# hkapp/cniic

Hardware: AMD Instinct MI355X
Metric: Mpixels/sec encode (cluster-colors K=256) (higher is better)
Workload: dtype u8/u64; 1 GPU; configs[1]: cluster-colors(256) encode of one 4096x4096 photo-like synthetic RGB image per GPU (seed 0x636E696963+2+rank), to convergence; image and stream HBM-resident; pixels_per_gpu=16777216, parallelism=1 GPU

## Files before the change

### cniic_amd/csrc/k_kmeans_persist.hip

```cpp
#include <atomic>

#include <hip/hip_ext.h>

#include "kmeans_rgbw.hpp"

namespace cniic {

constexpr int kPsThreads = 1024, kPsWaves = kPsThreads / 64;
constexpr uint32_t kPsAccWords = 5 * 256;
constexpr uint32_t kPsOffTab = kPsAccWords * 8, kPsOffS = kPsOffTab + 256 * 8;
static_assert(kPsOffCell == kPsOffS + kPsSlotsMax * kPsScap * 4, "ps_cell_bytes / kPsOffCell (kmeans_rgbw.hpp) describe this layout");

__device__ __forceinline__ uint32_t ps_xcc_id() {
    uint32_t v;
    asm volatile("s_getreg_b32 %0, hwreg(HW_REG_XCC_ID)" : "=s"(v));
    return v & 7u;
}
__device__ __forceinline__ unsigned long long ps_aread(unsigned long long *p) {
    return __hip_atomic_fetch_add(p, 0ull, __ATOMIC_RELAXED, __HIP_MEMORY_SCOPE_AGENT);
}
__device__ __forceinline__ uint32_t ps_ld(const uint32_t *p) { return __hip_atomic_load(p, __ATOMIC_RELAXED, __HIP_MEMORY_SCOPE_AGENT); }
__device__ __forceinline__ void ps_st(uint32_t *p, uint32_t v) { __hip_atomic_store(p, v, __ATOMIC_RELAXED, __HIP_MEMORY_SCOPE_AGENT); }

__device__ __forceinline__ bool ps_spin(uint32_t *word, uint32_t old, PsBar *b, unsigned long long ticks) {
    const unsigned long long t0 = wall_clock64();
    uint32_t spins = 0;
    while (ps_ld(word) == old) {
        __builtin_amdgcn_s_sleep(1);
        if ((++spins & 63u) == 0) {
            if (ps_ld(&b->abort_.v)) return false;
            if (wall_clock64() - t0 > ticks) { ps_st(&b->abort_.v, 1u); return false; }
        }
    }
    return true;
}
__device__ __forceinline__ bool ps_barrier_flat(PsBar *b, uint32_t nblocks, unsigned long long ticks) {
    const uint32_t g = ps_ld(&b->gen.v);
    if (__hip_atomic_fetch_add(&b->count.v, 1u, __ATOMIC_RELAXED, __HIP_MEMORY_SCOPE_AGENT) == nblocks - 1) {
        ps_st(&b->count.v, 0u);
        ps_st(&b->gen.v, g + 1);
        return true;
    }
    return ps_spin(&b->gen.v, g, b, ticks);
}
__device__ __forceinline__ bool ps_barrier_xcd(PsBar *b, uint32_t x, uint32_t nx_blocks, uint32_t nxcd, unsigned long long ticks) {
    const uint32_t tg = ps_ld(&b->topgen.v);
    if (__hip_atomic_fetch_add(&b->xcount[x].v, 1u, __ATOMIC_RELAXED, __HIP_MEMORY_SCOPE_AGENT) == nx_blocks - 1) {
        ps_st(&b->xcount[x].v, 0u);
        if (__hip_atomic_fetch_add(&b->top.v, 1u, __ATOMIC_RELAXED, __HIP_MEMORY_SCOPE_AGENT) == nxcd - 1) {
            ps_st(&b->top.v, 0u);
            ps_st(&b->topgen.v, tg + 1);
            return true;
        }
    }
    return ps_spin(&b->topgen.v, tg, b, ticks);
}

__global__ __launch_bounds__(1024) void k_ps_ranges(const uint32_t *__restrict__ ne_cost, const uint32_t *__restrict__ ne_count, uint32_t G, uint32_t dyn_bytes,
                                                    uint32_t *__restrict__ cb, uint32_t *__restrict__ fail) {
    const uint32_t M = *ne_count, NC = G * kPsChunks;
    const uint64_t total = ne_cost[M];
    for (uint32_t g0 = threadIdx.x; g0 <= NC; g0 += 8 * blockDim.x) {
        uint32_t a[8], b[8];
        uint64_t c_lo[8];
#pragma unroll
        for (int r = 0; r < 8; r++) {
            const uint32_t g = g0 + r * blockDim.x;
            c_lo[r] = total * min(g, NC) / NC;
            a[r] = 0; b[r] = g <= NC ? M : 0u;
        }
        bool more = true;
        while (more) {
            more = false;
            uint32_t mid[8], v[8];
#pragma unroll
            for (int r = 0; r < 8; r++) { mid[r] = (a[r] + b[r]) >> 1; v[r] = a[r] < b[r] ? ne_cost[mid[r]] : 0u; }
#pragma unroll
            for (int r = 0; r < 8; r++)
                if (a[r] < b[r]) { if (v[r] < c_lo[r]) a[r] = mid[r] + 1; else b[r] = mid[r]; more = more || a[r] < b[r]; }
        }
#pragma unroll
        for (int r = 0; r < 8; r++) {
            const uint32_t g = g0 + r * blockDim.x;
            if (g <= NC) cb[g] = g == NC ? M : a[r];
        }
    }
    __syncthreads();
    for (uint32_t g = threadIdx.x; g < G; g += blockDim.x) {
        uint32_t C = 0;
        for (uint32_t r = 0; r < kPsChunks; r++) C += cb[r * G + g + 1] - cb[r * G + g];
        if (C > kPsMaxCells || kPsOffCell + ps_cell_bytes(C) > dyn_bytes) atomicAdd(fail, 1u);
    }
}

template <class Op> __device__ __forceinline__ uint32_t row_allreduce(uint32_t v, Op op) {
    v = op(v, (uint32_t)__builtin_amdgcn_update_dpp(0, (int)v, 0x121, 0xf, 0xf, false));
    v = op(v, (uint32_t)__builtin_amdgcn_update_dpp(0, (int)v, 0x122, 0xf, 0xf, false));
    v = op(v, (uint32_t)__builtin_amdgcn_update_dpp(0, (int)v, 0x124, 0xf, 0xf, false));
    v = op(v, (uint32_t)__builtin_amdgcn_update_dpp(0, (int)v, 0x128, 0xf, 0xf, false));
    return v;
}
__device__ __forceinline__ uint32_t row_min(uint32_t v) { return row_allreduce(v, [](uint32_t a, uint32_t b) { return a < b ? a : b; }); }
__device__ __forceinline__ uint32_t row_max(uint32_t v) { return row_allreduce(v, [](uint32_t a, uint32_t b) { return a > b ? a : b; }); }
__device__ __forceinline__ uint32_t row_sum(uint32_t v) { return row_allreduce(v, [](uint32_t a, uint32_t b) { return a + b; }); }

__device__ __forceinline__ uint32_t ps_centre_dist(uint32_t ck, uint32_t cpk, uint32_t cc) { return dot4u8(ck, ck, cc) - 2u * dot4u8(ck, cpk, 0); }

__device__ __forceinline__ void ps_build_lists(const uint2 *tab, uint32_t K, uint32_t nslots, const uint16_t *ssup, uint32_t *s_nS, uint32_t *s_lpiv, uint32_t *Sent, int wid, int lane) {
    constexpr int32_t ext = (1 << (kCellShift + 2)) - 1;
    for (uint32_t slot = (uint32_t)wid; slot < nslots; slot += kPsWaves) {
        const CellBox bx = super_box((uint32_t)__builtin_amdgcn_readfirstlane((int)ssup[slot]));
        const uint32_t cpk = pack_rgb(bx.r0 + 16, bx.g0 + 16, bx.b0 + 16), cc = dot4u8(cpk, cpk, 0);
        uint32_t ck[4], best = 0xffffffffu;
#pragma unroll
        for (int r = 0; r < 4; r++) {
            const uint32_t k = 64u * r + (uint32_t)lane;
            ck[r] = k < K ? tab[k].x : 0u;
            if (k < K) best = min(best, (ps_centre_dist(ck[r], cpk, cc) << 8) | k);
        }
        const uint32_t piv = wave_reduce_min(best) & 255u;
        Dominance dm;
        dm.set(bx, ext, (uint32_t)__builtin_amdgcn_readfirstlane((int)tab[piv].x));
        uint32_t n = 0;
#pragma unroll
        for (int r = 0; r < 4; r++) {
            const uint32_t k = 64u * r + (uint32_t)lane;
            const bool keep = k < K && dm.worst(ck[r]) >= 0;
            const unsigned long long bm = __ballot(keep);
            const uint32_t pos = n + lanes_below(bm);
            if (keep && pos < kPsScap) Sent[slot * kPsScap + pos] = (k << 24) | ck[r];
            n += (uint32_t)__popcll(bm);
        }
        if (lane == 0) { s_nS[slot] = n; s_lpiv[slot] = piv; }
    }
    __syncthreads();
}

constexpr uint32_t kPsUlMask = 0x1ffu, kPsComplete = 0x200u;

__device__ __forceinline__ bool ps_row_finish(uint32_t *rec, uint32_t l16, uint32_t pid, uint32_t lpid, bool complete) {
    const uint32_t w = l16 < 8 ? rec[2 + l16] : 0u;
    const uint32_t pc = (uint32_t)__popc(w);
    uint32_t inc = pc;
    inc += (uint32_t)__builtin_amdgcn_update_dpp(0, (int)inc, 0x111, 0xf, 0xf, true);
    inc += (uint32_t)__builtin_amdgcn_update_dpp(0, (int)inc, 0x112, 0xf, 0xf, true);
    inc += (uint32_t)__builtin_amdgcn_update_dpp(0, (int)inc, 0x114, 0xf, 0xf, true);
    const uint32_t cnt = row_max(inc);
    uint32_t pos = inc - pc, ww = w;
    uint8_t *c4 = reinterpret_cast<uint8_t *>(rec + 10);
    while (ww && pos < 4) {
        c4[pos] = (uint8_t)(32u * l16 + (uint32_t)__builtin_ctz(ww));
        ww &= ww - 1;
        pos++;
    }
    const uint32_t r1 = rec[1];
    if (l16 == 0) rec[1] = (r1 & kPsUlMask) | (pid << 16) | (lpid << 24) | (complete ? kPsComplete : 0u);
    const uint32_t only = rec[10] & 255u;
    return !(cnt == 1 && (r1 & kPsUlMask) == only);
}

__device__ __forceinline__ uint32_t ps_row_build_list(const uint2 *tab, const uint32_t *ent, uint32_t n, uint32_t c, uint32_t l16, uint32_t *rec) {
    constexpr int32_t ext = (1 << kCellShift) - 1;
    constexpr int PER = kPsScap / 16;
    const CellBox bx = cell_box(c);
    const uint32_t cpk = pack_rgb(bx.r0 + 4, bx.g0 + 4, bx.b0 + 4), cc = dot4u8(cpk, cpk, 0);
    uint32_t en[PER];
#pragma unroll
    for (int t = 0; t < PER; t++) en[t] = l16 + 16u * t < n ? ent[l16 + 16u * t] : 0xffffffffu;
    uint32_t best = 0xffffffffu;
#pragma unroll
    for (int t = 0; t < PER; t++)
        if (l16 + 16u * t < n) best = min(best, (ps_centre_dist(en[t] & 0xffffffu, cpk, cc) << 8) | (en[t] >> 24));
    const uint32_t pid = row_min(best) & 255u;
    Dominance dm;
    dm.set(bx, ext, tab[pid].x);
    if (l16 < 8) rec[2 + l16] = 0u;
#pragma unroll
    for (int t = 0; t < PER; t++)
        if (l16 + 16u * t < n && dm.worst(en[t] & 0xffffffu) >= 0) { const uint32_t k = en[t] >> 24; atomicOr(&rec[2 + (k >> 5)], 1u << (k & 31)); }
    if (l16 == 0) rec[0] = tab[pid].x;
    return pid;
}
__device__ __forceinline__ uint32_t ps_row_build_table(const uint2 *tab, uint32_t K, uint32_t c, uint32_t l16, uint32_t *rec) {
    constexpr int32_t ext = (1 << kCellShift) - 1;
    const CellBox bx = cell_box(c);
    const uint32_t cpk = pack_rgb(bx.r0 + 4, bx.g0 + 4, bx.b0 + 4), cc = dot4u8(cpk, cpk, 0);
    uint32_t best = 0xffffffffu;
    for (uint32_t k = l16; k < K; k += 16) best = min(best, (ps_centre_dist(tab[k].x, cpk, cc) << 8) | k);
    const uint32_t pid = row_min(best) & 255u;
    Dominance dm;
    dm.set(bx, ext, tab[pid].x);
    if (l16 < 8) rec[2 + l16] = 0u;
    for (uint32_t k = l16; k < K; k += 16)
        if (dm.worst(tab[k].x) >= 0) atomicOr(&rec[2 + (k >> 5)], 1u << (k & 31));
    if (l16 == 0) rec[0] = tab[pid].x;
    return pid;
}

__device__ __forceinline__ void ps_best(const uint32_t (&key)[kSweep], const unsigned long long (&nm)[4], const uint2 *tab, uint32_t (&best)[kSweep]) {
#pragma unroll
    for (int u = 0; u < kSweep; u++) best[u] = 0;
#pragma unroll
    for (int w = 0; w < 4; w++) {
        unsigned long long mm = nm[w];
        while (mm) {
            const uint32_t k = 64 * w + (uint32_t)__builtin_ctzll(mm);
            mm &= mm - 1;
            const uint2 cc = tab[k];
#pragma unroll
            for (int u = 0; u < kSweep; u++) best[u] = max(best[u], (dot4u8(key[u], cc.x, 0) << 9) + cc.y);
        }
    }
}

__device__ __forceinline__ uint32_t ps_pack(uint32_t key, uint32_t w, uint32_t label) {
    const uint32_t wc = min(w, 255u);
    return (key & 0x070707u) | ((wc & 31u) << 3) | ((wc >> 5) << 11) | ((255u - label) << 24);
}
__device__ __forceinline__ uint32_t ps_wt(uint32_t w) { return ((w >> 3) & 31u) | ((w >> 6) & 0xe0u); }

__device__ __forceinline__ void ps_book_move(unsigned long long *acc, uint32_t K, uint32_t pp, uint64_t w, uint32_t ol, uint32_t nl) {
    const unsigned long long rw = ((pp >> 16) & 255) * w, gw = ((pp >> 8) & 255) * w, bw = (pp & 255) * w;
    atomicAdd(&acc[3 * nl + 0], rw); atomicAdd(&acc[3 * nl + 1], gw); atomicAdd(&acc[3 * nl + 2], bw);
    atomicAdd(&acc[3 * K + nl], (unsigned long long)w); atomicAdd(&acc[4 * K + nl], 1ull);
    atomicAdd(&acc[3 * ol + 0], 0ull - rw); atomicAdd(&acc[3 * ol + 1], 0ull - gw); atomicAdd(&acc[3 * ol + 2], 0ull - bw);
    atomicAdd(&acc[3 * K + ol], 0ull - (unsigned long long)w); atomicAdd(&acc[4 * K + ol], 0ull - 1ull);
}

__device__ __forceinline__ void ps_scores(const uint32_t (&key)[kSweep], const unsigned long long (&nm)[4], uint32_t ncand, uint32_t cand4, const uint2 *tab, uint32_t (&best)[kSweep]) {
    if (ncand <= 4) {
        const uint2 c0 = tab[cand4 & 255u], c1 = tab[(cand4 >> 8) & 255u], c2 = tab[(cand4 >> 16) & 255u], c3 = tab[cand4 >> 24];
#pragma unroll
        for (int u = 0; u < kSweep; u++) best[u] = (dot4u8(key[u], c0.x, 0) << 9) + c0.y;
        if (ncand > 1) {
#pragma unroll
            for (int u = 0; u < kSweep; u++) best[u] = max(best[u], (dot4u8(key[u], c1.x, 0) << 9) + c1.y);
        }
        if (ncand > 2) {
#pragma unroll
            for (int u = 0; u < kSweep; u++) best[u] = max(best[u], (dot4u8(key[u], c2.x, 0) << 9) + c2.y);
        }
        if (ncand > 3) {
#pragma unroll
            for (int u = 0; u < kSweep; u++) best[u] = max(best[u], (dot4u8(key[u], c3.x, 0) << 9) + c3.y);
        }
    } else ps_best(key, nm, tab, best);
}

template <typename StoreLabel>
__device__ __forceinline__ bool ps_sweep(const uint32_t (&wd)[kSweep], uint32_t base, uint32_t e, uint32_t s0, int lane, const unsigned long long (&nm)[4], uint32_t ncand,
                                         uint32_t cand4, const uint2 *tab, uint32_t K, uint32_t cbk, const uint32_t *__restrict__ cwq, unsigned long long *acc, uint32_t &moved,
                                         bool agg, StoreLabel store_label) {
    uint32_t key[kSweep], lc[kSweep];
    bool valid[kSweep];
#pragma unroll
    for (int u = 0; u < kSweep; u++) {
        key[u] = cbk | (wd[u] & 0x070707u);
        lc[u] = wd[u] >> 24;
        valid[u] = base + u * 64 + lane < e;
    }
    if (ncand == 1) {
        const uint32_t onlyc = 255u - (cand4 & 255u);
        bool same = true;
#pragma unroll
        for (int u = 0; u < kSweep; u++) same = same & (!valid[u] | (lc[u] == onlyc));
        if (__ballot(!same) == 0ull) return true;
    }
    uint32_t best[kSweep];
    ps_scores(key, nm, ncand, cand4, tab, best);
    bool mv[kSweep], any = false;
#pragma unroll
    for (int u = 0; u < kSweep; u++) { mv[u] = valid[u] & ((best[u] & 255u) != lc[u]); any = any | mv[u]; }
    if (!__ballot(any)) return false;
    any = false;
#pragma unroll
    for (int u = 0; u < kSweep; u++) {
        const uint2 cc = tab[255u - lc[u]];
        const uint32_t kc = (dot4u8(key[u], cc.x, 0) << 9) + cc.y;
        mv[u] = mv[u] & ((best[u] >> 8) > (kc >> 8));
        any = any | mv[u];
    }
    if (!__ballot(any)) return false;
    uint32_t wt[kSweep];
    bool heavy = false;
#pragma unroll
    for (int u = 0; u < kSweep; u++) { wt[u] = ps_wt(wd[u]); heavy = heavy | (mv[u] & (wt[u] == 255u)); }
    if (__ballot(heavy)) {
#pragma unroll
        for (int u = 0; u < kSweep; u++)
            if (mv[u] && wt[u] == 255u) wt[u] = cwq[base + u * 64 + lane - s0];
    }
#pragma unroll
    for (int u = 0; u < kSweep; u++)
        if (mv[u]) { store_label(base + u * 64 + lane, best[u] & 255u); moved++; }
    if (agg) {
        static_assert(kSweep == 4, "four slots per lane");
        uint32_t nmv = 0;
#pragma unroll
        for (int u = 0; u < kSweep; u++) nmv += (uint32_t)__popcll(__ballot(mv[u]));
        if (nmv >= kAggMin) {
#pragma unroll 1
            for (int round = 0; round < 6; round++) {
                const unsigned long long b0 = __ballot(mv[0]), b1 = __ballot(mv[1]), b2 = __ballot(mv[2]), b3 = __ballot(mv[3]);
                if (!(b0 | b1 | b2 | b3)) return false;
                uint32_t pn, po;
                if (b0) { const int l = __builtin_ctzll(b0); pn = (uint32_t)__builtin_amdgcn_readlane((int)best[0], l) & 255u; po = (uint32_t)__builtin_amdgcn_readlane((int)lc[0], l); }
                else if (b1) { const int l = __builtin_ctzll(b1); pn = (uint32_t)__builtin_amdgcn_readlane((int)best[1], l) & 255u; po = (uint32_t)__builtin_amdgcn_readlane((int)lc[1], l); }
                else if (b2) { const int l = __builtin_ctzll(b2); pn = (uint32_t)__builtin_amdgcn_readlane((int)best[2], l) & 255u; po = (uint32_t)__builtin_amdgcn_readlane((int)lc[2], l); }
                else { const int l = __builtin_ctzll(b3); pn = (uint32_t)__builtin_amdgcn_readlane((int)best[3], l) & 255u; po = (uint32_t)__builtin_amdgcn_readlane((int)lc[3], l); }
                uint32_t cnt = 0;
                bool mt[kSweep];
#pragma unroll
                for (int u = 0; u < kSweep; u++) {
                    mt[u] = mv[u] && (best[u] & 255u) == pn && lc[u] == po;
                    cnt += (uint32_t)__popcll(__ballot(mt[u]));
                    mv[u] = mv[u] && !mt[u];
                }
                if (cnt < kAggMin) {
#pragma unroll
                    for (int u = 0; u < kSweep; u++) mv[u] = mv[u] || mt[u];
                    break;
                }
                const size_t kn = 255u - pn, ko = 255u - po;
                auto book = [&](int shift, uint32_t mask, size_t at_new, size_t at_old) {
                    unsigned long long v = 0;
#pragma unroll
                    for (int u = 0; u < kSweep; u++)
                        if (mt[u]) v += (unsigned long long)(mask ? (key[u] >> shift) & mask : 1u) * wt[u];
                    v = wave_reduce_sum64(v);
                    if (lane == 0) { atomicAdd(&acc[at_new], v); atomicAdd(&acc[at_old], 0ull - v); }
                };
                book(16, 255u, 3 * kn + 0, 3 * ko + 0);
                book(8, 255u, 3 * kn + 1, 3 * ko + 1);
                book(0, 255u, 3 * kn + 2, 3 * ko + 2);
                book(0, 0u, 3 * (size_t)K + kn, 3 * (size_t)K + ko);
                if (lane == 0) { atomicAdd(&acc[4 * K + kn], (unsigned long long)cnt); atomicAdd(&acc[4 * K + ko], 0ull - (unsigned long long)cnt); }
            }
        }
    }
    for (;;) {
        const bool has = mv[0] | mv[1] | mv[2] | mv[3];
        if (!__ballot(has)) break;
        if (has) {
            const int u = mv[0] ? 0 : mv[1] ? 1 : mv[2] ? 2 : 3;
            const uint32_t kk = u == 0 ? key[0] : u == 1 ? key[1] : u == 2 ? key[2] : key[3];
            const uint32_t ww = u == 0 ? wt[0] : u == 1 ? wt[1] : u == 2 ? wt[2] : wt[3];
            const uint32_t bb = u == 0 ? best[0] : u == 1 ? best[1] : u == 2 ? best[2] : best[3];
            const uint32_t oo = u == 0 ? lc[0] : u == 1 ? lc[1] : u == 2 ? lc[2] : lc[3];
            ps_book_move(acc, K, kk, ww, 255u - oo, 255u - (bb & 255u));
            mv[0] = mv[0] & (u != 0); mv[1] = mv[1] & (u != 1); mv[2] = mv[2] & (u != 2); mv[3] = false | (mv[3] & (u != 3));
        }
    }
    return false;
}

template <typename StoreLabel>
__device__ __forceinline__ void ps_sweep_first(const uint32_t (&wd)[kSweep], uint32_t base, uint32_t e, uint32_t s0, int lane, const unsigned long long (&nm)[4], uint32_t ncand,
                                               uint32_t cand4, const uint2 *tab, uint32_t K, uint32_t cbk, const uint32_t *__restrict__ cwq, unsigned long long *acc, uint32_t &moved,
                                               StoreLabel store_label) {
    uint32_t p[kSweep], lc[kSweep], wt[kSweep];
    bool heavy = false;
#pragma unroll
    for (int u = 0; u < kSweep; u++) {
        p[u] = cbk | (wd[u] & 0x070707u);
        lc[u] = wd[u] >> 24;
        wt[u] = ps_wt(wd[u]);
        heavy = heavy | (wt[u] == 255u);
    }
    if (__ballot(heavy)) {
#pragma unroll
        for (int u = 0; u < kSweep; u++)
            if (wt[u] == 255u && base + u * 64 + lane < e) wt[u] = cwq[base + u * 64 + lane - s0];
    }
    uint32_t best[kSweep];
    ps_scores(p, nm, ncand, cand4, tab, best);
    uint32_t nl[kSweep];
    bool rem[kSweep];
#pragma unroll
    for (int u = 0; u < kSweep; u++) {
        const uint32_t idx = base + u * 64 + lane;
        nl[u] = lc[u];
        rem[u] = idx < e;
        if (rem[u] && (best[u] & 255u) != lc[u]) {
            const uint2 cc = tab[255u - lc[u]];
            const uint32_t kc = (dot4u8(p[u], cc.x, 0) << 9) + cc.y;
            if ((best[u] >> 8) > (kc >> 8)) { nl[u] = best[u] & 255u; moved++; store_label(idx, nl[u]); }
        }
    }
    static_assert(kSweep == 4, "four slots per lane");
#pragma unroll 1
    for (int round = 0; round < 6; round++) {
        const unsigned long long b0 = __ballot(rem[0]), b1 = __ballot(rem[1]), b2 = __ballot(rem[2]), b3 = __ballot(rem[3]);
        if (!(b0 | b1 | b2 | b3)) return;
        uint32_t pn;
        if (b0) pn = (uint32_t)__builtin_amdgcn_readlane((int)nl[0], __builtin_ctzll(b0));
        else if (b1) pn = (uint32_t)__builtin_amdgcn_readlane((int)nl[1], __builtin_ctzll(b1));
        else if (b2) pn = (uint32_t)__builtin_amdgcn_readlane((int)nl[2], __builtin_ctzll(b2));
        else pn = (uint32_t)__builtin_amdgcn_readlane((int)nl[3], __builtin_ctzll(b3));
        uint32_t cnt = 0, mbits = 0;
#pragma unroll
        for (int u = 0; u < kSweep; u++) {
            const bool match = rem[u] && nl[u] == pn;
            mbits |= match ? 1u << u : 0u;
            cnt += (uint32_t)__popcll(__ballot(match));
            rem[u] = rem[u] && !match;
        }
        const size_t kn = 255u - pn;
        auto book = [&](int shift, uint32_t mask, size_t at) {
            unsigned long long v = 0;
#pragma unroll
            for (int u = 0; u < kSweep; u++)
                if ((mbits >> u) & 1u) v += (unsigned long long)(mask ? (p[u] >> shift) & mask : 1u) * wt[u];
            v = wave_reduce_sum64(v);
            if (lane == 0) atomicAdd(&acc[at], v);
        };
        book(16, 255u, 3 * kn + 0);
        book(8, 255u, 3 * kn + 1);
        book(0, 255u, 3 * kn + 2);
        book(0, 0u, 3 * (size_t)K + kn);
        if (lane == 0) atomicAdd(&acc[4 * K + kn], (unsigned long long)cnt);
    }
#pragma unroll
    for (int u = 0; u < kSweep; u++) {
        if (rem[u]) {
            const uint32_t pp = p[u], n_ = 255u - nl[u];
            const uint64_t w = wt[u];
            atomicAdd(&acc[3 * n_ + 0], ((pp >> 16) & 255) * w); atomicAdd(&acc[3 * n_ + 1], ((pp >> 8) & 255) * w); atomicAdd(&acc[3 * n_ + 2], (pp & 255) * w);
            atomicAdd(&acc[3 * K + n_], (unsigned long long)w); atomicAdd(&acc[4 * K + n_], 1ull);
        }
    }
}

struct PsCold {
    PsExit exit;
    uint2 *cconst_g;
    uint32_t *cent_g;
    uint64_t *members_out, *wsum_out;
    const uint32_t *keys;
    GIdx gx;
    uint64_t seed, U;
};
struct PsArgs {
    const uint32_t *ckeys, *cweight;
    uint8_t *labels;
    const uint32_t *ne_cell, *ne_start;
    const uint32_t *cb;
    const uint32_t *ranges_fail;
    uint32_t *pk;
    const uint2 *cconst0;
    unsigned long long *partials;
    PsBar *bar;
    KmDevState *st_rw;
    PsCold *cold;
    uint64_t max_iters;
    uint32_t K, max_skip, agg_iters, test_abort_at, lds_budget;
    uint32_t clean_skip;
    unsigned long long timeout_ticks;
};

__global__ __launch_bounds__(kPsThreads) void k_rgbw_persist(PsArgs a) {
    extern __shared__ __align__(16) unsigned long long lds[];
    __shared__ uint32_t s_moved, s_nmoved, s_reseed, s_active, s_ok, s_nx, s_nxcd, s_qn, s_qhead, s_Cres, s_nslots;
    __shared__ uint32_t s_mlist[kMaxMovedSkip];
    __shared__ unsigned long long s_mm[4], s_evals, s_changed, s_pev;
    __shared__ uint32_t s_nS[kPsSlotsMax], s_lpiv[kPsSlotsMax], s_mcol[kMaxMovedSkip];
    __shared__ uint16_t s_ssup[kPsSlotsMax];
    __shared__ uint32_t s_cbase[kPsChunks + 1], s_cm0[kPsChunks], s_scan[kPsThreads / 64];
    const uint32_t tid = threadIdx.x, K = a.K, G = gridDim.x;
    const int lane = tid & 63, wid = tid >> 6;
    unsigned long long *acc = lds;
    uint2 *tab = reinterpret_cast<uint2 *>(reinterpret_cast<uint8_t *>(lds) + kPsOffTab);
    uint32_t *Sent = reinterpret_cast<uint32_t *>(reinterpret_cast<uint8_t *>(lds) + kPsOffS);
    if (*a.ranges_fail) {
        if (blockIdx.x == 0 && tid == 0) { a.cold->exit.status = kPsStatusRanges; __threadfence_system(); }
        return;
    }
    if (tid < kPsChunks) {
        const uint32_t m0 = a.cb[tid * G + blockIdx.x], m1 = a.cb[tid * G + blockIdx.x + 1];
        s_cm0[tid] = m0;
        s_cbase[tid + 1] = m1 - m0;
    }
    if (tid == 0) {
        s_cbase[0] = 0;
        s_moved = 0; s_evals = 0; s_nmoved = 0; s_reseed = 0; s_active = 0; s_mm[0] = s_mm[1] = s_mm[2] = s_mm[3] = 0ull; s_qn = 0; s_qhead = 0; s_Cres = 0; s_nslots = 0;
    }
    __syncthreads();
    if (tid == 0)
        for (uint32_t r = 0; r < kPsChunks; r++) s_cbase[r + 1] += s_cbase[r];
    __syncthreads();
    const uint32_t C = s_cbase[kPsChunks], Cr = (C + 3u) & ~3u;
    uint8_t *cellb = reinterpret_cast<uint8_t *>(lds) + kPsOffCell;
    uint32_t *cstart = reinterpret_cast<uint32_t *>(cellb);
    uint32_t *gstart = cstart + Cr + 4;
    uint32_t *recs = gstart + Cr;
    uint16_t *ccell = reinterpret_cast<uint16_t *>(recs + (size_t)kPsRecWords * Cr);
    uint16_t *queue = ccell + Cr;
    uint8_t *cslot = reinterpret_cast<uint8_t *>(queue + Cr);
    uint32_t *pts = reinterpret_cast<uint32_t *>(cslot + Cr);
    const uint32_t cap = (a.lds_budget - kPsOffCell - ps_cell_bytes(C)) / 4u;
    {
        uint32_t np[2] = {0, 0}, cid[2] = {0, 0}, rr[2] = {0, 0};
        bool mine[2];
#pragma unroll
        for (int q = 0; q < 2; q++) {
            const uint32_t i = 2 * tid + q;
            mine[q] = i < C;
            if (mine[q]) {
                uint32_t r = 0;
                while (i >= s_cbase[r + 1]) r++;
                rr[q] = r;
                const uint32_t m = s_cm0[r] + (i - s_cbase[r]);
                cid[q] = a.ne_cell[m];
                const uint32_t gs = a.ne_start[m];
                np[q] = a.ne_start[m + 1] - gs;
                ccell[i] = (uint16_t)cid[q];
                gstart[i] = gs;
                uint32_t *rec = recs + (size_t)kPsRecWords * i;
                rec[0] = 0u; rec[1] = kPsUlMask; rec[10] = 0u;
            }
        }
        const uint32_t off = block_exclusive_scan<kPsThreads>(np[0] + np[1], s_scan);
        if (mine[0]) cstart[2 * tid] = off;
        if (mine[1]) cstart[2 * tid + 1] = off + np[0];
        if (tid == (C ? (C - 1) / 2 : 0)) cstart[C] = C ? off + np[0] + np[1] : 0u;
        __syncthreads();
        bool flag[2];
#pragma unroll
        for (int q = 0; q < 2; q++) {
            const uint32_t i = 2 * tid + q;
            flag[q] = mine[q] && (i == s_cbase[rr[q]] || ((uint32_t)ccell[i - 1] >> kSuperShift) != (cid[q] >> kSuperShift));
        }
        const uint32_t before = block_exclusive_scan<kPsThreads>((flag[0] ? 1u : 0u) + (flag[1] ? 1u : 0u), s_scan);
        uint32_t run_f = before;
#pragma unroll
        for (int q = 0; q < 2; q++) {
            const uint32_t i = 2 * tid + q;
            run_f += flag[q] ? 1u : 0u;
            if (mine[q]) {
                const uint32_t sidx = run_f - 1u;
                cslot[i] = sidx < kPsSlotsMax ? (uint8_t)sidx : (uint8_t)255;
                if (flag[q] && sidx < kPsSlotsMax) s_ssup[sidx] = (uint16_t)(cid[q] >> kSuperShift);
                if (i == C - 1) s_nslots = min(sidx + 1u, kPsSlotsMax);
                if (cstart[i + 1] <= cap && (i + 1 == C || cstart[i + 2] > cap)) s_Cres = i + 1;
            }
        }
    }
    for (uint32_t i = tid; i < 5 * K; i += kPsThreads) acc[i] = 0ull;
    for (uint32_t i = tid; i < K; i += kPsThreads) tab[i] = a.cconst0[i];
    __syncthreads();
    {
        const uint32_t Cres0 = s_Cres;
        for (uint32_t i = wid; i < C; i += kPsWaves) {
            const uint32_t s = cstart[i], n = cstart[i + 1] - s, gs = gstart[i];
            const uint32_t cbk = cell_base_key(ccell[i]);
            (void)cbk;
            for (uint32_t t0 = 0; t0 < n; t0 += 256) {
                uint32_t kk[4], ww[4], ll[4];
#pragma unroll
                for (int u = 0; u < 4; u++) {
                    const uint32_t t = t0 + u * 64 + lane;
                    const bool in = t < n;
                    kk[u] = in ? a.ckeys[gs + t] : 0u;
                    ww[u] = in ? a.cweight[gs + t] : 0u;
                    ll[u] = in ? (uint32_t)a.labels[gs + t] : 0u;
                }
#pragma unroll
                for (int u = 0; u < 4; u++) {
                    const uint32_t t = t0 + u * 64 + lane;
                    if (t < n) {
                        const uint32_t w = ps_pack(kk[u], ww[u], ll[u]);
                        if (i < Cres0) pts[s + t] = w; else a.pk[gs + t] = w;
                    }
                }
            }
        }
    }
    if (tid == 0) {
        const uint32_t x = ps_xcc_id();
        __hip_atomic_fetch_add(&a.bar->xblocks[x].v, 1u, __ATOMIC_RELAXED, __HIP_MEMORY_SCOPE_AGENT);
        const bool ok = ps_barrier_flat(a.bar, G, a.timeout_ticks);
        uint32_t n = 0;
        for (int i = 0; i < 8; i++) n += ps_ld(&a.bar->xblocks[i].v) != 0;
        s_nx = ps_ld(&a.bar->xblocks[x].v);
        s_nxcd = n;
        s_ok = ok;
    }
    __syncthreads();
    if (!s_ok) {
        if (tid == 0) { a.cold->exit.status = kPsStatusAborted; __threadfence_system(); }
        return;
    }
    const uint32_t Cres = s_Cres, nslots = s_nslots;
    const uint32_t row = (uint32_t)lane >> 4, l16 = (uint32_t)lane & 15u;
    unsigned long long run[5] = {0, 0, 0, 0, 0};
    uint32_t moved = 0;
    unsigned long long evals = 0;
    uint32_t j = 0;
    uint32_t nS = K;
    unsigned long long reseeds_total = 0, evals_total = 0;
    for (;;) {
        const bool first = j == 0;
        const bool skip_mode = !first && a.max_skip && nS <= a.max_skip;
        if (!skip_mode) {
            ps_build_lists(tab, K, nslots, s_ssup, s_nS, s_lpiv, Sent, wid, lane);
            for (uint32_t i0 = (uint32_t)wid * 4; i0 < C; i0 += kPsWaves * 4) {
                const uint32_t i = i0 + row;
                if (i < C) {
                    const uint32_t c = ccell[i], slot = cslot[i];
                    const uint32_t nl = slot != 255u ? s_nS[slot] : 0xffffffffu;
                    uint32_t *rec = recs + (size_t)kPsRecWords * i;
                    const uint32_t w_old = l16 < 8 ? rec[2 + l16] : 0u;
                    bool needs;
                    if (nl <= kPsScap) {
                        const uint32_t pid = ps_row_build_list(tab, Sent + slot * kPsScap, nl, c, l16, rec);
                        needs = ps_row_finish(rec, l16, pid, s_lpiv[slot], false);
                    } else {
                        const uint32_t pid = ps_row_build_table(tab, K, c, l16, rec);
                        needs = ps_row_finish(rec, l16, pid, 0u, true);
                    }
                    if (!first && a.clean_skip) {
                        const uint32_t mm32 = l16 < 8 ? (uint32_t)(s_mm[l16 >> 1] >> (32u * (l16 & 1u))) : 0u;
                        const uint32_t w_new = l16 < 8 ? rec[2 + l16] : 0u;
                        needs = needs && row_max(((w_old | w_new) & mm32) ? 1u : 0u) != 0u;
                    }
                    if (l16 == 0 && (needs || first)) queue[atomicAdd(&s_qn, 1u)] = (uint16_t)i;
                }
            }
        } else {
            uint32_t mk[4], mc[4];
#pragma unroll
            for (int t = 0; t < 4; t++) {
                const uint32_t jj = l16 + 16u * t;
                mk[t] = jj < nS ? s_mlist[jj] : 0xffffffffu;
                mc[t] = jj < nS ? s_mcol[jj] : 0u;
            }
            for (uint32_t i0 = (uint32_t)wid * 4; i0 < C; i0 += kPsWaves * 4) {
                const uint32_t i = i0 + row;
                const bool ok = i < C;
                const uint32_t *rec = recs + (size_t)kPsRecWords * (ok ? i : 0u);
                const uint32_t r1 = rec[1], lp = r1 >> 24, c = ccell[ok ? i : 0u];
                Dominance dm;
                dm.set(cell_box(c), (1 << kCellShift) - 1, rec[0]);
                bool dv = !(r1 & kPsComplete) && ((s_mm[lp >> 6] >> (lp & 63)) & 1ull) != 0ull;
#pragma unroll
                for (int t = 0; t < 4; t++) {
                    if (mk[t] != 0xffffffffu) {
                        const bool in = ((rec[2 + (mk[t] >> 5)] >> (mk[t] & 31)) & 1u) != 0;
                        dv = dv | in | (dm.worst(mc[t]) >= 0);
                    }
                }
                const unsigned long long bm = __ballot(dv && ok);
                if (l16 == 0 && ((bm >> (16 * row)) & 0xffffull)) queue[atomicAdd(&s_qn, 1u)] = (uint16_t)i;
            }
        }
        __syncthreads();
        {
            const uint32_t qn = s_qn;
            const bool agg = !first && j <= a.agg_iters;
            for (;;) {
                uint32_t qi = 0;
                if (lane == 0) qi = atomicAdd(&s_qhead, 1u);
                qi = (uint32_t)__builtin_amdgcn_readfirstlane((int)qi);
                if (qi >= qn) break;
                const uint32_t i = queue[qi];
                const uint32_t s = cstart[i], e = cstart[i + 1], gs = gstart[i], c = ccell[i];
                uint32_t rw = lane < (int)kPsRecWords ? recs[(size_t)kPsRecWords * i + lane] : 0u;
                if (skip_mode) {
                    constexpr int32_t ext = (1 << kCellShift) - 1;
                    const uint32_t r1o = (uint32_t)__builtin_amdgcn_readlane((int)rw, 1), pido = (r1o >> 16) & 255u, lpo = r1o >> 24;
                    const bool keep = ((s_mm[pido >> 6] >> (pido & 63)) & 1ull) == 0ull && ((r1o & kPsComplete) || ((s_mm[lpo >> 6] >> (lpo & 63)) & 1ull) == 0ull);
                    const CellBox bx = cell_box(c);
                    unsigned long long um[4];
                    uint32_t npid = pido, npv = (uint32_t)__builtin_amdgcn_readlane((int)rw, 0);
                    bool complete = (r1o & kPsComplete) != 0;
                    if (keep) {
                        Dominance dm;
                        dm.set(bx, ext, npv);
                        const uint32_t k1 = (uint32_t)lane < nS ? s_mlist[lane] : 0xffffffffu;
                        const uint32_t ck1 = (uint32_t)lane < nS ? s_mcol[lane] : 0u;
                        unsigned long long f1 = __ballot(k1 != 0xffffffffu && dm.worst(ck1) >= 0);
#pragma unroll
                        for (int w = 0; w < 4; w++)
                            um[w] = (((unsigned long long)(uint32_t)__builtin_amdgcn_readlane((int)rw, 3 + 2 * w) << 32) | (uint32_t)__builtin_amdgcn_readlane((int)rw, 2 + 2 * w)) & ~s_mm[w];
                        while (f1) {
                            const int l = __builtin_ctzll(f1);
                            f1 &= f1 - 1;
                            const uint32_t k = (uint32_t)__builtin_amdgcn_readlane((int)k1, l);
                            const unsigned long long bit = 1ull << (k & 63);
                            const uint32_t w = (k >> 6) & 3;
                            um[0] |= w == 0 ? bit : 0ull; um[1] |= w == 1 ? bit : 0ull; um[2] |= w == 2 ? bit : 0ull; um[3] |= w == 3 ? bit : 0ull;
                        }
                    } else {
                        npid = nearest_to_centre(tab, K, bx, ext, lane);
                        npv = (uint32_t)__builtin_amdgcn_readfirstlane((int)tab[npid].x);
                        Dominance dm;
                        dm.set(bx, ext, npv);
#pragma unroll
                        for (int w = 0; w < 4; w++) {
                            const uint32_t k = 64 * w + lane;
                            um[w] = __ballot(k < K && dm.worst(tab[k < K ? k : 0].x) >= 0);
                        }
                        complete = true;
                    }
#pragma unroll
                    for (int w = 0; w < 4; w++) um[w] = ((unsigned long long)(uint32_t)__builtin_amdgcn_readfirstlane((int)(uint32_t)(um[w] >> 32)) << 32) | (uint32_t)__builtin_amdgcn_readfirstlane((int)(uint32_t)um[w]);
                    uint32_t c4 = 0, got = 0;
                    {
                        unsigned long long t4[4] = {um[0], um[1], um[2], um[3]};
#pragma unroll
                        for (int w = 0; w < 4; w++)
                            while (t4[w] && got < 4) { c4 |= (64u * w + (uint32_t)__builtin_ctzll(t4[w])) << (8 * got); t4[w] &= t4[w] - 1; got++; }
                    }
                    const uint32_t r1n = (r1o & kPsUlMask) | (npid << 16) | (complete ? kPsComplete : (r1o & 0xff000000u));
                    uint32_t nw = rw;
#pragma unroll
                    for (int t = 0; t < 8; t++)
                        if (lane == 2 + t) nw = (uint32_t)(um[t >> 1] >> (32 * (t & 1)));
                    if (lane == 0) nw = npv;
                    if (lane == 1) nw = r1n;
                    if (lane == 10) nw = c4;
                    rw = nw;
                    if (lane < (int)kPsRecWords) recs[(size_t)kPsRecWords * i + lane] = rw;
                    const uint32_t ncd = (uint32_t)(__popcll(um[0]) + __popcll(um[1]) + __popcll(um[2]) + __popcll(um[3]));
                    if (ncd == 1 && (r1o & kPsUlMask) == (c4 & 255u)) continue;
                }
                uint32_t wd[kSweep];
                if (i < Cres) {
#pragma unroll
                    for (int u = 0; u < kSweep; u++) { const uint32_t idx = s + u * 64 + lane; wd[u] = idx < e ? pts[idx] : 0u; }
                } else {
#pragma unroll
                    for (int u = 0; u < kSweep; u++) { const uint32_t idx = s + u * 64 + lane; wd[u] = idx < e ? a.pk[gs + (idx - s)] : 0u; }
                }
                unsigned long long nm[4];
#pragma unroll
                for (int w = 0; w < 4; w++)
                    nm[w] = ((unsigned long long)(uint32_t)__builtin_amdgcn_readlane((int)rw, 3 + 2 * w) << 32) | (uint32_t)__builtin_amdgcn_readlane((int)rw, 2 + 2 * w);
                const uint32_t r1 = (uint32_t)__builtin_amdgcn_readlane((int)rw, 1), cand4 = (uint32_t)__builtin_amdgcn_readlane((int)rw, 10);
                const uint32_t ncand = (uint32_t)(__popcll(nm[0]) + __popcll(nm[1]) + __popcll(nm[2]) + __popcll(nm[3]));
                const uint32_t cbk = cell_base_key(c);
                const bool res = i < Cres;
                const uint32_t *cwc = a.cweight + gs;
                uint32_t *pkc = a.pk + gs;
                uint32_t *rec = recs + (size_t)kPsRecWords * i;
                bool uniform = !first;
                for (uint32_t base = s; base < e; base += 64 * kSweep) {
                    uint32_t w2[kSweep] = {0, 0, 0, 0};
                    if (base + 64 * kSweep < e) {
                        if (res) {
#pragma unroll
                            for (int u = 0; u < kSweep; u++) { const uint32_t idx = base + 64 * kSweep + u * 64 + lane; w2[u] = idx < e ? pts[idx] : 0u; }
                        } else {
#pragma unroll
                            for (int u = 0; u < kSweep; u++) { const uint32_t idx = base + 64 * kSweep + u * 64 + lane; w2[u] = idx < e ? pkc[idx - s] : 0u; }
                        }
                    }
                    if (res) {
                        auto st = [&](uint32_t idx, uint32_t l) { reinterpret_cast<uint8_t *>(pts)[4 * idx + 3] = (uint8_t)l; };
                        if (first) ps_sweep_first(wd, base, e, s, lane, nm, ncand, cand4, tab, K, cbk, cwc, acc, moved, st);
                        else uniform = ps_sweep(wd, base, e, s, lane, nm, ncand, cand4, tab, K, cbk, cwc, acc, moved, agg, st) && uniform;
                    } else {
                        auto st = [&](uint32_t idx, uint32_t l) { reinterpret_cast<uint8_t *>(pkc)[4 * (size_t)(idx - s) + 3] = (uint8_t)l; };
                        if (first) ps_sweep_first(wd, base, e, s, lane, nm, ncand, cand4, tab, K, cbk, cwc, acc, moved, st);
                        else uniform = ps_sweep(wd, base, e, s, lane, nm, ncand, cand4, tab, K, cbk, cwc, acc, moved, agg, st) && uniform;
                    }
#pragma unroll
                    for (int u = 0; u < kSweep; u++) wd[u] = w2[u];
                }
                if (lane == 0) rec[1] = (r1 & ~kPsUlMask) | (uniform && ncand == 1 ? cand4 & 255u : kPsUlMask);
                evals += (unsigned long long)(e - s) * (ncand + 1);
            }
        }
        moved = wave_reduce_sum(moved);
        if (lane == 0) {
            if (moved) atomicAdd(&s_moved, moved);
            if (evals) atomicAdd(&s_evals, evals);
        }
        moved = 0; evals = 0;
        __syncthreads();
        unsigned long long *Pcur = a.partials + (size_t)(j % 3) * kPsPartWords;
        for (uint32_t i = tid; i < 5 * K; i += kPsThreads) {
            const unsigned long long v = acc[i];
            if (v) { __hip_atomic_fetch_add(&Pcur[i], v, __ATOMIC_RELAXED, __HIP_MEMORY_SCOPE_AGENT); acc[i] = 0ull; }
        }
        if (tid == 0) {
            if (s_moved) __hip_atomic_fetch_add(&Pcur[5 * (size_t)K], (unsigned long long)s_moved, __ATOMIC_RELAXED, __HIP_MEMORY_SCOPE_AGENT);
            if (s_evals) __hip_atomic_fetch_add(&Pcur[5 * (size_t)K + 1], s_evals, __ATOMIC_RELAXED, __HIP_MEMORY_SCOPE_AGENT);
            s_moved = 0; s_evals = 0; s_qn = 0; s_qhead = 0; s_nmoved = 0; s_reseed = 0; s_active = 0; s_mm[0] = s_mm[1] = s_mm[2] = s_mm[3] = 0ull;
        }
        asm volatile("s_waitcnt vmcnt(0)" ::: "memory");
        __syncthreads();
        if (tid == 0) {
            bool ok = ps_barrier_xcd(a.bar, ps_xcc_id(), s_nx, s_nxcd, a.timeout_ticks);
#ifdef CNIIC_TESTING
            if (a.test_abort_at && j + 1 == a.test_abort_at) { ps_st(&a.bar->abort_.v, 1u); ok = false; }
#endif
            s_ok = ok;
        }
        __syncthreads();
        if (!s_ok) {
            if (tid == 0) { a.cold->exit.status = kPsStatusAborted; __threadfence_system(); }
            return;
        }
        j++;
        if (blockIdx.x == 0) {
            unsigned long long *Pclr = a.partials + (size_t)((j + 1) % 3) * kPsPartWords;
            for (uint32_t i = tid; i < 5 * K + 2; i += kPsThreads) __hip_atomic_store(&Pclr[i], 0ull, __ATOMIC_RELAXED, __HIP_MEMORY_SCOPE_AGENT);
        }
        if (tid < K) {
            const uint32_t k = tid;
            const size_t at[5] = {3 * (size_t)k, 3 * (size_t)k + 1, 3 * (size_t)k + 2, 3 * (size_t)K + k, 4 * (size_t)K + k};
            unsigned long long d[5];
#pragma unroll
            for (int i = 0; i < 5; i++) d[i] = ps_aread(&Pcur[at[i]]);
#pragma unroll
            for (int i = 0; i < 5; i++) run[i] += d[i];
            uint32_t ck;
            if (run[4] == 0) {
                const PsCold *cd = a.cold;
                const uint64_t ri = reseed_index(cd->seed, j - 1, k, cd->U);
                const GIdx gx = cd->gx;
                ck = gx.bits ? gidx_select(gx, ri) : cd->keys[ri];
                atomicAdd(&s_reseed, 1u);
            } else {
                const uint32_t r = div_floor_small(run[0], run[3]) & 255, g = div_floor_small(run[1], run[3]) & 255, b = div_floor_small(run[2], run[3]) & 255;
                ck = (r << 16) | (g << 8) | b;
                atomicAdd(&s_active, 1u);
            }
            const uint32_t oldc = tab[k].x;
            tab[k] = make_cconst(ck, k, 8);
            if (ck != oldc) {
                const uint32_t pos = atomicAdd(&s_nmoved, 1u);
                if (pos < kMaxMovedSkip) { s_mlist[pos] = k; s_mcol[pos] = ck; }
                atomicOr(&s_mm[(k >> 6) & 3], 1ull << (k & 63));
            }
        } else if (tid == kPsThreads - 1) {
            s_changed = ps_aread(&Pcur[5 * (size_t)K]);
            s_pev = ps_aread(&Pcur[5 * (size_t)K + 1]);
        }
        __syncthreads();
        const unsigned long long changed = s_changed;
        nS = s_nmoved;
        reseeds_total += s_reseed;
        evals_total += s_pev;
        const bool fin = changed == 0 || (a.max_iters && j >= a.max_iters);
        if (blockIdx.x == 0 && tid == 0) {
            KmDevState *sw = a.st_rw;
            sw->changed_ring[(j - 1) % kHistRing] = changed;
            sw->nmoved_ring[(j - 1) % kHistRing] = nS;
            if (fin) {
                sw->moved_last = changed; sw->reseeds = reseeds_total; sw->active = s_active; sw->pair_evals = evals_total; sw->iter = j; sw->done = 1;
                PsExit *x = &a.cold->exit;
                x->iter = j; x->moved_last = changed; x->reseeds = reseeds_total; x->active = s_active; x->pair_evals = evals_total;
            }
        }
        if (fin) break;
    }
    if (blockIdx.x == 0 && tid < K) {
        const PsCold *cd = a.cold;
        const uint2 cc = tab[tid];
        cd->cent_g[tid] = cc.x;
        cd->cconst_g[tid] = cc;
        cd->members_out[tid] = run[4];
        cd->wsum_out[tid] = run[3];
    }
    for (uint32_t i = wid; i < C; i += kPsWaves) {
        const uint32_t s = cstart[i], n = cstart[i + 1] - s, gs = gstart[i];
        if (i < Cres) { for (uint32_t t = lane; t < n; t += 64) a.labels[gs + t] = (uint8_t)(255u - (pts[s + t] >> 24)); }
        else { for (uint32_t t = lane; t < n; t += 64) a.labels[gs + t] = (uint8_t)(255u - (a.pk[gs + t] >> 24)); }
    }
    if (blockIdx.x == 0) {
        __syncthreads();
        if (tid == 0) { __threadfence_system(); a.cold->exit.status = kPsStatusDone; __threadfence_system(); }
    }
}

static std::atomic<int> g_ps_cus_in_use[16];

static int ps_cu_count(int device) {
    static std::atomic<int> cached[16];
    const int d = device >= 0 && device < 16 ? device : 0;
    int n = cached[d].load();
    if (n) return n;
    hipDeviceProp_t prop;
    if (hipGetDeviceProperties(&prop, device) != hipSuccess) { (void)hipGetLastError(); return 0; }
    cached[d].store(prop.multiProcessorCount);
    return prop.multiProcessorCount;
}

uint32_t ps_grid_for(Ctx *c, uint64_t Umax) {
    uint32_t G = (uint32_t)ps_cu_count(c->device);
    if (!G) return 0;
    G = std::max(1u, G / std::max(1u, c->ps_div));
    if (const uint64_t mb = c->opt(CNIIC_OPT_KM_MAX_BLOCKS, "CNIIC_KM_MAX_BLOCKS", 0)) G = std::max<uint32_t>(1u, (uint32_t)((uint64_t)G * std::min<uint64_t>(mb, 768) / 768));
    if (const char *e = test_env("CNIIC_KM_PS_BLOCKS")) G = std::max(1, atoi(e));
    G = (uint32_t)std::min<uint64_t>(G, std::max<uint64_t>(1, ceil_div(Umax, 512)));
    return std::min<uint32_t>(G, 1024u);
}

static void ps_learn(Ctx *c, uint32_t status, bool injected) {
    if (status == kPsStatusDone) { c->ps_backoff = 0; c->ps_backoff_left = 0; return; }
    if (status != kPsStatusAborted || injected) return;
    c->ps_backoff = std::min<uint32_t>(256u, std::max<uint32_t>(4u, 2u * c->ps_backoff));
    c->ps_backoff_left = c->ps_backoff;
}

int ps_prepare(KmRgbwState *s) {
    Ctx *c = s->c;
    if (c->ps_backoff_left && !test_env("CNIIC_KM_PS_REQUIRE")) { c->ps_backoff_left--; return CNIIC_OK; }
    const uint32_t G = ps_grid_for(c, s->U);
    if (!G) return CNIIC_OK;
    static bool attr_set[16] = {};
    if (c->device >= 0 && c->device < 16 && !attr_set[c->device]) {
        CNIIC_HIP_TRY(c, hipFuncSetAttribute(reinterpret_cast<const void *>(k_rgbw_persist), hipFuncAttributeMaxDynamicSharedMemorySize, (int)kPsDynBytes));
        attr_set[c->device] = true;
    }
    const uint64_t o_bar = 0, o_part = (sizeof(PsBar) + 255) & ~255ull, o_fail = o_part + ((3 * (uint64_t)kPsPartWords * 8 + 255) & ~255ull);
    const uint64_t o_rng = o_fail + 256, total = o_rng + ((uint64_t)G * kPsChunks + 1) * 4;
    CNIIC_HIP_TRY(c, s->ps_arena.alloc(total));
    CNIIC_HIP_TRY(c, hipMemsetAsync(s->ps_arena.p, 0, o_rng, c->stream));
    CNIIC_HIP_TRY(c, s->ps_pk.alloc(std::max<uint64_t>(s->U, 1) * 4));
    s->ps_blocks = G;
    s->ps_o_part = o_part; s->ps_o_fail = o_fail; s->ps_o_rng = o_rng;
    (void)o_bar;
    uint8_t *a = s->ps_arena.as<uint8_t>();
    uint32_t budget = kPsDynBytes;
    if (const char *e = test_env("CNIIC_TEST_PS_LDS_BYTES")) budget = std::min<uint32_t>(kPsDynBytes, (uint32_t)atoi(e));
    s->ps_budget = budget;
    hipLaunchKernelGGL(k_ps_ranges, dim3(1), dim3(1024), 0, c->stream, (const uint32_t *)s->ne_cost.as<uint32_t>(), (const uint32_t *)s->ne_count.as<uint32_t>(), G, budget,
                       reinterpret_cast<uint32_t *>(a + o_rng), reinterpret_cast<uint32_t *>(a + o_fail));
    CNIIC_HIP_TRY(c, hipGetLastError());
    s->ps = true;
    return CNIIC_OK;
}

int km_rgbw_run_persistent(KmRgbwState *s, bool *ran, bool may_defer) {
    Ctx *c = s->c;
    *ran = false;
    if (!s->ps || s->ps_tried) return CNIIC_OK;
    s->ps_tried = true;
    const int dev = c->device >= 0 && c->device < 16 ? c->device : 0, G = (int)s->ps_blocks;
    if (g_ps_cus_in_use[dev].fetch_add(G) + G > ps_cu_count(c->device)) { g_ps_cus_in_use[dev].fetch_sub(G); return CNIIC_OK; }
    std::shared_ptr<void> release(nullptr, [dev, G](void *) { g_ps_cus_in_use[dev].fetch_sub(G); });
    CNIIC_HIP_TRY(c, c->pinned_ps.reserve(1024, 1024));
    static_assert(sizeof(PsCold) <= 1024, "the pinned block holds a PsCold");
    PsCold *cold = c->pinned_ps.as<PsCold>();
    memset(cold, 0, sizeof *cold);
    PsExit *xh = &cold->exit;
    uint8_t *ar = s->ps_arena.as<uint8_t>();
    PsArgs a{};
    a.ckeys = s->ckeys.as<uint32_t>(); a.cweight = s->cweight.as<uint32_t>(); a.labels = s->labels.as<uint8_t>();
    a.ne_cell = s->ne_cell.as<uint32_t>(); a.ne_start = s->ne_start.as<uint32_t>();
    a.cb = reinterpret_cast<const uint32_t *>(ar + s->ps_o_rng); a.ranges_fail = reinterpret_cast<const uint32_t *>(ar + s->ps_o_fail);
    a.lds_budget = s->ps_budget;
    a.pk = s->ps_pk.as<uint32_t>(); a.cconst0 = s->cconst.as<uint2>();
    a.partials = reinterpret_cast<unsigned long long *>(ar + s->ps_o_part); a.bar = reinterpret_cast<PsBar *>(ar);
    cold->cconst_g = s->cconst.as<uint2>(); cold->cent_g = s->cent.as<uint32_t>(); cold->members_out = s->members_last.as<uint64_t>(); cold->wsum_out = s->wsum_last.as<uint64_t>();
    cold->keys = s->keys; cold->gx = s->gidx; cold->seed = s->seed; cold->U = s->gidx.bits ? s->gidx.U : s->U;
    a.st_rw = s->dstate.as<KmDevState>(); a.cold = cold; a.max_iters = s->max_iters;
    a.K = s->K; a.max_skip = s->no_skip ? 0u : s->max_skip; a.agg_iters = kAggLaunches;
    a.test_abort_at = 0;
    if (const char *e = test_env("CNIIC_TEST_PS_ABORT_AT")) a.test_abort_at = (uint32_t)atoi(e);
    a.clean_skip = 1;
    if (const char *e = test_env("CNIIC_KM_PS_CLEANSKIP")) a.clean_skip = atoi(e) ? 1u : 0u;
    uint64_t tmo_ms = 2000;
    if (const char *e = test_env("CNIIC_KM_PS_TIMEOUT_MS")) tmo_ms = (uint64_t)atoll(e);
    a.timeout_ticks = tmo_ms * 100000ull;
    hipEvent_t e0 = nullptr, e1 = nullptr;
    if (s->profile) { CNIIC_HIP_TRY(c, hipEventCreate(&e0)); CNIIC_HIP_TRY(c, hipEventCreate(&e1)); }
    hipExtLaunchKernelGGL(k_rgbw_persist, dim3((uint32_t)G), dim3(kPsThreads), kPsDynBytes, c->stream, e0, e1, 0, a);
    CNIIC_HIP_TRY(c, hipGetLastError());
    if (may_defer && !s->profile) {
        s->ps_pending = true;
        s->ps_hold = release;
        *ran = true;
        return CNIIC_OK;
    }
    CNIIC_HIP_TRY(c, ctx_spin_sync(c));
    const uint32_t status = xh->status;
    ps_learn(c, status, a.test_abort_at != 0);
    if (status != kPsStatusDone) {
        if (e0) { (void)hipEventDestroy(e0); (void)hipEventDestroy(e1); }
        if (test_env("CNIIC_KM_PS_REQUIRE")) return c->fail(CNIIC_ERR_HIP, "kmeans_rgbw: the persistent launch ended with status %u (CNIIC_KM_PS_REQUIRE)", status);
        return CNIIC_OK;
    }
    s->run_stats.iterations = xh->iter; s->run_stats.moved_last = xh->moved_last; s->run_stats.empty_reseeds = xh->reseeds;
    s->run_stats.active = xh->active; s->run_stats.pair_evals = xh->pair_evals;
    s->run_stats_valid = true;
    if (s->profile) {
        float ms = 0.f;
        (void)hipEventElapsedTime(&ms, e0, e1);
        (void)hipEventDestroy(e0); (void)hipEventDestroy(e1);
        KernelTime &kt = c->ktimes["kmeans_rgbw_persist"];
        kt.ms += ms; kt.launches += 1;
        KernelTime &ki = c->ktimes["kmeans_rgbw_persist_iters"];
        ki.ms += ms; ki.launches += xh->iter;
    }
    *ran = true;
    return CNIIC_OK;
}

int km_rgbw_persistent_verdict(KmRgbwState *s, bool *retry) {
    Ctx *c = s->c;
    *retry = false;
    s->ps_pending = false;
    s->ps_hold.reset();
    const PsExit *xh = &c->pinned_ps.as<const PsCold>()->exit;
    ps_learn(c, xh->status, test_env("CNIIC_TEST_PS_ABORT_AT") != nullptr);
    if (xh->status == kPsStatusDone) {
        s->run_stats.iterations = xh->iter; s->run_stats.moved_last = xh->moved_last; s->run_stats.empty_reseeds = xh->reseeds;
        s->run_stats.active = xh->active; s->run_stats.pair_evals = xh->pair_evals;
        s->run_stats_valid = true;
        return CNIIC_OK;
    }
    if (test_env("CNIIC_KM_PS_REQUIRE")) return c->fail(CNIIC_ERR_HIP, "kmeans_rgbw: the persistent launch ended with status %u (CNIIC_KM_PS_REQUIRE)", xh->status);
    CNIIC_TRY(km_rgbw_run(s, nullptr, false));
    *retry = true;
    return CNIIC_OK;
}

}
```

### cniic_amd/csrc/kmeans_rgbw.hpp

```cpp
#pragma once
#include <cstdlib>
#include <memory>
#include <vector>

#include "common.hpp"
#include "device_utils.hpp"

namespace cniic {

constexpr uint32_t kBias = 1u << 18;
constexpr int kPPT = 8;
constexpr int kAssignThreads = 256;
constexpr uint32_t kMaxBlocks = 512;
constexpr int kCellWaves = 8;
__host__ __device__ constexpr uint32_t km_scap(uint32_t K) { return K <= 256 ? (K + 1) / 2 : (K + 1) / 2 < 512u ? (K + 1) / 2 : 512u; }
__host__ __device__ constexpr uint32_t km_ccap(uint32_t K) { return K <= 256 ? K : 256u; }
constexpr uint32_t kCellWavesBig = 12;
constexpr uint32_t kBigBlocksFrom = 10;
constexpr uint32_t kAggLaunches = 3;
constexpr uint32_t kCellBlocks = 256 * 3;
constexpr int kSweep = 4;
constexpr uint32_t kCellFixedCost = 512;
constexpr uint32_t kCellSweepCost = 256;

struct KmRgbwState {
    Ctx *c = nullptr;
    uint64_t U = 0, lo = 0, hi = 0, seed = 0, max_iters = 0;
    uint32_t K = 0, Kpad = 0, idbits = 8, nblocks = 1;
    bool wide = false;
    bool big = false;
    bool cells = true;
    bool profile = false;
    bool no_skip = false;
    const uint32_t *keys = nullptr, *weight = nullptr;
    DevBuf labels;
    DevBuf cconst, slabs, partials_own, dstate, cent, members_last, wsum_last;
    DevBuf arena;
    DevBuf resblk;
    uint64_t res_cent = 0, res_members = 0, res_wsum = 0, res_bytes = 0;
    std::unique_ptr<LaggedPoll> lagged;
    DevBuf ckeys, cweight, crank, cell_start, running, ne_cell, ne_start, ne_cost, ne_count, wfirst;
    DevBuf cell_rec, moved_list;
    uint32_t wfirst_waves = 0;
    GIdx gidx{nullptr, nullptr, 0};
    DevBuf fused_partials, fused_running, fused_cent;
    bool fused = false;
    cniic_kmeans_stats run_stats{};
    bool run_stats_valid = false;
    uint32_t max_skip = 64;
    long fail_at = -1;
    uint32_t shard = 0, nshards = 1;
    uint64_t *partials = nullptr;
    bool ps = false, ps_tried = false;
    bool ps_pending = false;
    std::shared_ptr<void> ps_hold;
    uint32_t ps_blocks = 0;
    DevBuf ps_arena;
    DevBuf ps_pk;
    uint64_t ps_o_part = 0, ps_o_fail = 0, ps_o_rng = 0;
    uint32_t ps_budget = 0;
    bool started = false;
    DevBuf given;
    std::vector<uint32_t> given_h;
};

constexpr uint32_t kPsChunks = 24;
constexpr uint32_t kPsSlotsMax = 32;
constexpr uint32_t kPsScap = 96;
constexpr uint32_t kPsRecWords = 11;
constexpr uint32_t kPsMaxCells = 2048;
constexpr uint32_t kPsOffCell = 5 * 256 * 8 + 256 * 8 + kPsSlotsMax * kPsScap * 4;
constexpr uint32_t kPsDynBytes = 160 * 1024 - 3072;
constexpr uint32_t kPsPartWords = 5 * 256 + 8;
__host__ __device__ constexpr uint32_t ps_cell_bytes(uint32_t C) { return 16u + ((C + 3u) & ~3u) * (4u + 4u + kPsRecWords * 4u + 2u + 2u + 1u); }
struct alignas(128) PsLine { uint32_t v; uint32_t pad[31]; };
struct PsBar { PsLine xcount[8], xgen[8], xblocks[8], top, topgen, count, gen, abort_; };
constexpr uint32_t kPsStatusDone = 1, kPsStatusAborted = 2, kPsStatusRanges = 3;
struct PsExit { uint32_t status, pad; uint64_t iter, moved_last, reseeds, active, pair_evals; };
void launch_rgbw_assign_big(Ctx *c, const uint32_t *ckeys, const uint32_t *cweight, uint64_t U, uint32_t K, const uint32_t *cent, uint16_t *labels,
                            unsigned long long *partials, const KmDevState *st);
int ps_prepare(KmRgbwState *s);
int km_rgbw_run_persistent(KmRgbwState *s, bool *ran, bool may_defer);
int km_rgbw_persistent_verdict(KmRgbwState *s, bool *retry);
constexpr uint32_t kAggMin = 16;


__device__ __forceinline__ uint32_t dot4u8(uint32_t a, uint32_t b, uint32_t acc) {
    return __builtin_amdgcn_udot4(a, b, acc, false);
}

__device__ __forceinline__ uint2 make_cconst(uint32_t ckey, uint32_t k, uint32_t idbits) {
    uint32_t h = dot4u8(ckey, ckey, 0);
    uint32_t idmask = (1u << idbits) - 1;
    return make_uint2(ckey, ((kBias - h) << idbits) | (idmask - k));
}

struct CellBox { int32_t r0, g0, b0; };
__device__ __forceinline__ CellBox super_box(uint32_t sup) {
    return CellBox{(int32_t)((sup / (kSupersPerDim * kSupersPerDim)) << (kCellShift + 2)),
                   (int32_t)(((sup / kSupersPerDim) % kSupersPerDim) << (kCellShift + 2)),
                   (int32_t)((sup % kSupersPerDim) << (kCellShift + 2))};
}
__device__ __forceinline__ CellBox cell_box(uint32_t c) {
    const CellBox sb = super_box(c >> kSuperShift);
    return CellBox{sb.r0 + (int32_t)(((c >> 4) & 3) << kCellShift), sb.g0 + (int32_t)(((c >> 2) & 3) << kCellShift),
                   sb.b0 + (int32_t)((c & 3) << kCellShift)};
}

constexpr uint32_t kRecComplete = 0x80000000u;
__host__ __device__ constexpr uint32_t cell_rec_words(uint32_t MW) { return (2 + 2 * MW + 15) & ~15u; }
constexpr uint32_t kMaxMovedSkip = 64;

__device__ __forceinline__ uint32_t pack_rgb(int32_t r, int32_t g, int32_t b) { return ((uint32_t)r << 16) | ((uint32_t)g << 8) | (uint32_t)b; }

__device__ __forceinline__ uint32_t centre_dist(uint32_t ck, const CellBox &bx, int32_t ext) {
    const int32_t h = (ext + 1) >> 1;
    const uint32_t c = pack_rgb(bx.r0 + h, bx.g0 + h, bx.b0 + h);
    return dot4u8(ck, ck, dot4u8(c, c, 0)) - 2u * dot4u8(ck, c, 0);
}

struct Dominance {
    uint32_t ppk, lopk, hipk;
    int32_t cp, ext;
    __device__ __forceinline__ void set(const CellBox &bx, int32_t e, uint32_t pivot) {
        ppk = pivot & 0xffffffu;
        ext = e;
        lopk = pack_rgb(bx.r0, bx.g0, bx.b0);
        hipk = pack_rgb(bx.r0 + e, bx.g0 + e, bx.b0 + e);
        cp = (int32_t)dot4u8(ppk, ppk, 0) - 2 * (int32_t)dot4u8(ppk, lopk, 0) - e * (int32_t)dot4u8(ppk, 0x010101u, 0);
    }
    __device__ __forceinline__ int32_t worst(uint32_t ck) const {
        const uint32_t v = ck;
        return cp - (int32_t)dot4u8(v, v, 0) + (int32_t)dot4u8(v, hipk, dot4u8(v, lopk, 0)) + __mul24(ext, (int32_t)__builtin_amdgcn_sad_u8(ppk, v, 0u));
    }
};

__device__ __forceinline__ uint32_t wave_all_min(uint32_t v) { return wave_reduce_min(v); }

__device__ __forceinline__ uint32_t nearest_to_centre(const uint2 *list, uint32_t n, const CellBox &bx, int32_t ext, int lane) {
    uint32_t bd = 0xfffffu, be = 4095u;
    for (uint32_t e = lane; e < n; e += 64) {
        const uint32_t d = centre_dist(list[e].x, bx, ext);
        if (d < bd) { bd = d; be = e; }
    }
    return wave_all_min((bd << 12) | be) & 4095u;
}

__device__ __forceinline__ uint32_t lanes_below(unsigned long long bm) {
    return __builtin_amdgcn_mbcnt_hi((uint32_t)(bm >> 32), __builtin_amdgcn_mbcnt_lo((uint32_t)bm, 0u));
}

__device__ __forceinline__ uint32_t build_super(const uint2 *tab, uint32_t K, uint32_t sup, int lane, unsigned long long lt_mask,
                                                uint2 *S, uint32_t cap) {
    constexpr int32_t ext = (1 << (kCellShift + 2)) - 1;
    const CellBox bx = super_box(sup);
    Dominance dm;
    dm.set(bx, ext, tab[nearest_to_centre(tab, K, bx, ext, lane)].x);
    uint32_t n = 0;
    for (uint32_t k0 = 0; k0 < K; k0 += 64) {
        const uint32_t k = k0 + lane;
        uint2 cc = make_uint2(0u, 0u);
        bool keep = false;
        if (k < K) { cc = tab[k]; keep = dm.worst(cc.x) >= 0; }
        const unsigned long long bm = __ballot(keep);
        const uint32_t pos = n + lanes_below(bm);
        if (keep && pos < cap) S[pos] = cc;
        n += (uint32_t)__popcll(bm);
    }
    __builtin_amdgcn_wave_barrier();
    return n;
}

__device__ __forceinline__ uint32_t pk_make(uint32_t key, uint32_t w, uint32_t label) {
    return (((key >> 16) & 7u) << 6) | (((key >> 8) & 7u) << 3) | (key & 7u) | (min(w, 255u) << 16) | (label << 24);
}
__device__ __forceinline__ uint32_t pk_key(uint32_t pw, uint32_t cell_base) {
    return cell_base | ((pw & 0x1c0u) << 10) | ((pw & 0x38u) << 5) | (pw & 7u);
}
__device__ __forceinline__ uint32_t cell_base_key(uint32_t c) {
    const CellBox b = cell_box(c);
    return ((uint32_t)b.r0 << 16) | ((uint32_t)b.g0 << 8) | (uint32_t)b.b0;
}

}
```

Measured before the change: 10040 Mpixels/s.

## Move persistent kernel pointers and run totals out of registers into device arena and LDS

Moves rarely used global pointers from the kernel argument struct into a device-side PsDev record that the ranges kernel writes, and derives partials, ranges and fail addresses from the barrier arena base. Per-thread run accumulators and the reseed/eval totals move into LDS, and the skip-mode mlist/mcol preload is replaced by in-loop LDS reads. The loop also re-derives lane and wave ids through an opaque asm so the compiler does not keep them live. The aim is to cut SGPR/VGPR pressure in the persistent kernel. In exchange the resident-point LDS budget shrinks by 10 KiB and there are extra indirect loads.

```diff
diff --git a/cniic_amd/csrc/k_kmeans_persist.hip b/cniic_amd/csrc/k_kmeans_persist.hip
--- a/cniic_amd/csrc/k_kmeans_persist.hip
+++ b/cniic_amd/csrc/k_kmeans_persist.hip
@@ -9,6 +9,8 @@
 constexpr int kPsThreads = 1024, kPsWaves = kPsThreads / 64;
 constexpr uint32_t kPsAccWords = 5 * 256;
 constexpr uint32_t kPsOffTab = kPsAccWords * 8, kPsOffS = kPsOffTab + 256 * 8;
+constexpr uint32_t kPsStaticMax = 3072;
+static_assert(kPsDynBytes + kPsStaticMax <= 160 * 1024, "static + dynamic LDS of k_rgbw_persist: a CU has 160 KiB");
 static_assert(kPsOffCell == kPsOffS + kPsSlotsMax * kPsScap * 4, "ps_cell_bytes / kPsOffCell (kmeans_rgbw.hpp) describe this layout");
 
 __device__ __forceinline__ uint32_t ps_xcc_id() {
@@ -57,7 +59,9 @@
 }
 
 __global__ __launch_bounds__(1024) void k_ps_ranges(const uint32_t *__restrict__ ne_cost, const uint32_t *__restrict__ ne_count, uint32_t G, uint32_t dyn_bytes,
-                                                    uint32_t *__restrict__ cb, uint32_t *__restrict__ fail) {
+                                                    uint32_t *__restrict__ cb, PsDev *__restrict__ dev, PsDevPtrs ptrs) {
+    uint32_t *fail = &dev->fail;
+    if (threadIdx.x == 0) dev->p = ptrs;
     const uint32_t M = *ne_count, NC = G * kPsChunks;
     const uint64_t total = ne_cost[M];
     for (uint32_t g0 = threadIdx.x; g0 <= NC; g0 += 8 * blockDim.x) {
@@ -441,14 +445,8 @@
     uint64_t seed, U;
 };
 struct PsArgs {
-    const uint32_t *ckeys, *cweight;
-    uint8_t *labels;
-    const uint32_t *ne_cell, *ne_start;
-    const uint32_t *cb;
-    const uint32_t *ranges_fail;
+    const uint32_t *cweight;
     uint32_t *pk;
-    const uint2 *cconst0;
-    unsigned long long *partials;
     PsBar *bar;
     KmDevState *st_rw;
     PsCold *cold;
@@ -458,31 +456,39 @@
     unsigned long long timeout_ticks;
 };
 
+__device__ __forceinline__ unsigned long long *ps_partials(PsBar *bar) {
+    return reinterpret_cast<unsigned long long *>(reinterpret_cast<uint8_t *>(bar) + kPsArenaPart);
+}
+
 __global__ __launch_bounds__(kPsThreads) void k_rgbw_persist(PsArgs a) {
     extern __shared__ __align__(16) unsigned long long lds[];
     __shared__ uint32_t s_moved, s_nmoved, s_reseed, s_active, s_ok, s_nx, s_nxcd, s_qn, s_qhead, s_Cres, s_nslots;
     __shared__ uint32_t s_mlist[kMaxMovedSkip];
-    __shared__ unsigned long long s_mm[4], s_evals, s_changed, s_pev;
+    __shared__ unsigned long long s_mm[4], s_evals, s_changed, s_pev, s_rtot, s_etot;
     __shared__ uint32_t s_nS[kPsSlotsMax], s_lpiv[kPsSlotsMax], s_mcol[kMaxMovedSkip];
     __shared__ uint16_t s_ssup[kPsSlotsMax];
     __shared__ uint32_t s_cbase[kPsChunks + 1], s_cm0[kPsChunks], s_scan[kPsThreads / 64];
+    static_assert(4 * (11 + 2 * kMaxMovedSkip + 2 * kPsSlotsMax + 2 * kPsChunks + 1 + kPsThreads / 64) + 8 * (4 + 5) + 2 * kPsSlotsMax + 64 <= kPsStaticMax, "the static LDS of k_rgbw_persist");
     const uint32_t tid = threadIdx.x, K = a.K, G = gridDim.x;
     const int lane = tid & 63, wid = tid >> 6;
     unsigned long long *acc = lds;
+    unsigned long long *runs = lds + kPsBudget / 8;
     uint2 *tab = reinterpret_cast<uint2 *>(reinterpret_cast<uint8_t *>(lds) + kPsOffTab);
     uint32_t *Sent = reinterpret_cast<uint32_t *>(reinterpret_cast<uint8_t *>(lds) + kPsOffS);
-    if (*a.ranges_fail) {
+    const PsDev *dev = reinterpret_cast<const PsDev *>(reinterpret_cast<const uint8_t *>(a.bar) + kPsArenaFail);
+    if (dev->fail) {
         if (blockIdx.x == 0 && tid == 0) { a.cold->exit.status = kPsStatusRanges; __threadfence_system(); }
         return;
     }
     if (tid < kPsChunks) {
-        const uint32_t m0 = a.cb[tid * G + blockIdx.x], m1 = a.cb[tid * G + blockIdx.x + 1];
+        const uint32_t *cb = reinterpret_cast<const uint32_t *>(reinterpret_cast<const uint8_t *>(a.bar) + kPsArenaRng);
+        const uint32_t m0 = cb[tid * G + blockIdx.x], m1 = cb[tid * G + blockIdx.x + 1];
         s_cm0[tid] = m0;
         s_cbase[tid + 1] = m1 - m0;
     }
     if (tid == 0) {
         s_cbase[0] = 0;
-        s_moved = 0; s_evals = 0; s_nmoved = 0; s_reseed = 0; s_active = 0; s_mm[0] = s_mm[1] = s_mm[2] = s_mm[3] = 0ull; s_qn = 0; s_qhead = 0; s_Cres = 0; s_nslots = 0;
+        s_moved = 0; s_evals = 0; s_nmoved = 0; s_reseed = 0; s_active = 0; s_mm[0] = s_mm[1] = s_mm[2] = s_mm[3] = 0ull; s_qn = 0; s_qhead = 0; s_Cres = 0; s_nslots = 0; s_rtot = 0ull; s_etot = 0ull;
     }
     __syncthreads();
     if (tid == 0)
@@ -499,6 +505,7 @@
     uint32_t *pts = reinterpret_cast<uint32_t *>(cslot + Cr);
     const uint32_t cap = (a.lds_budget - kPsOffCell - ps_cell_bytes(C)) / 4u;
     {
+        const uint32_t *ne_cell = dev->p.ne_cell, *ne_start = dev->p.ne_start;
         uint32_t np[2] = {0, 0}, cid[2] = {0, 0}, rr[2] = {0, 0};
         bool mine[2];
 #pragma unroll
@@ -510,9 +517,9 @@
                 while (i >= s_cbase[r + 1]) r++;
                 rr[q] = r;
                 const uint32_t m = s_cm0[r] + (i - s_cbase[r]);
-                cid[q] = a.ne_cell[m];
-                const uint32_t gs = a.ne_start[m];
-                np[q] = a.ne_start[m + 1] - gs;
+                cid[q] = ne_cell[m];
+                const uint32_t gs = ne_start[m];
+                np[q] = ne_start[m + 1] - gs;
                 ccell[i] = (uint16_t)cid[q];
                 gstart[i] = gs;
                 uint32_t *rec = recs + (size_t)kPsRecWords * i;
@@ -546,10 +553,16 @@
         }
     }
     for (uint32_t i = tid; i < 5 * K; i += kPsThreads) acc[i] = 0ull;
-    for (uint32_t i = tid; i < K; i += kPsThreads) tab[i] = a.cconst0[i];
+    for (uint32_t i = tid; i < kPsRunWords; i += kPsThreads) runs[i] = 0ull;
+    {
+        const uint2 *cconst0 = dev->p.cconst0;
+        for (uint32_t i = tid; i < K; i += kPsThreads) tab[i] = cconst0[i];
+    }
     __syncthreads();
     {
         const uint32_t Cres0 = s_Cres;
+        const uint32_t *ckeys = dev->p.ckeys, *cweight = dev->p.cweight;
+        const uint8_t *labels0 = dev->p.labels;
         for (uint32_t i = wid; i < C; i += kPsWaves) {
             const uint32_t s = cstart[i], n = cstart[i + 1] - s, gs = gstart[i];
             const uint32_t cbk = cell_base_key(ccell[i]);
@@ -560,9 +573,9 @@
                 for (int u = 0; u < 4; u++) {
                     const uint32_t t = t0 + u * 64 + lane;
                     const bool in = t < n;
-                    kk[u] = in ? a.ckeys[gs + t] : 0u;
-                    ww[u] = in ? a.cweight[gs + t] : 0u;
-                    ll[u] = in ? (uint32_t)a.labels[gs + t] : 0u;
+                    kk[u] = in ? ckeys[gs + t] : 0u;
+                    ww[u] = in ? cweight[gs + t] : 0u;
+                    ll[u] = in ? (uint32_t)labels0[gs + t] : 0u;
                 }
 #pragma unroll
                 for (int u = 0; u < 4; u++) {
@@ -591,19 +604,20 @@
         return;
     }
     const uint32_t Cres = s_Cres, nslots = s_nslots;
-    const uint32_t row = (uint32_t)lane >> 4, l16 = (uint32_t)lane & 15u;
-    unsigned long long run[5] = {0, 0, 0, 0, 0};
     uint32_t moved = 0;
     unsigned long long evals = 0;
     uint32_t j = 0;
     uint32_t nS = K;
-    unsigned long long reseeds_total = 0, evals_total = 0;
     for (;;) {
+        uint32_t tid_i = threadIdx.x;
+        asm volatile("" : "+v"(tid_i));
+        const int lane_i = (int)(tid_i & 63u), wid_i = (int)(tid_i >> 6);
+        const uint32_t row = (uint32_t)lane_i >> 4, l16 = (uint32_t)lane_i & 15u;
         const bool first = j == 0;
         const bool skip_mode = !first && a.max_skip && nS <= a.max_skip;
         if (!skip_mode) {
-            ps_build_lists(tab, K, nslots, s_ssup, s_nS, s_lpiv, Sent, wid, lane);
-            for (uint32_t i0 = (uint32_t)wid * 4; i0 < C; i0 += kPsWaves * 4) {
+            ps_build_lists(tab, K, nslots, s_ssup, s_nS, s_lpiv, Sent, wid_i, lane_i);
+            for (uint32_t i0 = (uint32_t)wid_i * 4; i0 < C; i0 += kPsWaves * 4) {
                 const uint32_t i = i0 + row;
                 if (i < C) {
                     const uint32_t c = ccell[i], slot = cslot[i];
@@ -627,14 +641,7 @@
                 }
             }
         } else {
-            uint32_t mk[4], mc[4];
-#pragma unroll
-            for (int t = 0; t < 4; t++) {
-                const uint32_t jj = l16 + 16u * t;
-                mk[t] = jj < nS ? s_mlist[jj] : 0xffffffffu;
-                mc[t] = jj < nS ? s_mcol[jj] : 0u;
-            }
-            for (uint32_t i0 = (uint32_t)wid * 4; i0 < C; i0 += kPsWaves * 4) {
+            for (uint32_t i0 = (uint32_t)wid_i * 4; i0 < C; i0 += kPsWaves * 4) {
                 const uint32_t i = i0 + row;
                 const bool ok = i < C;
                 const uint32_t *rec = recs + (size_t)kPsRecWords * (ok ? i : 0u);
@@ -644,9 +651,11 @@
                 bool dv = !(r1 & kPsComplete) && ((s_mm[lp >> 6] >> (lp & 63)) & 1ull) != 0ull;
 #pragma unroll
                 for (int t = 0; t < 4; t++) {
-                    if (mk[t] != 0xffffffffu) {
-                        const bool in = ((rec[2 + (mk[t] >> 5)] >> (mk[t] & 31)) & 1u) != 0;
-                        dv = dv | in | (dm.worst(mc[t]) >= 0);
+                    const uint32_t jj = l16 + 16u * t;
+                    if (jj < nS) {
+                        const uint32_t mk = s_mlist[jj], mc = s_mcol[jj];
+                        const bool in = ((rec[2 + (mk >> 5)] >> (mk & 31)) & 1u) != 0;
+                        dv = dv | in | (dm.worst(mc) >= 0);
                     }
                 }
                 const unsigned long long bm = __ballot(dv && ok);
@@ -659,12 +668,12 @@
             const bool agg = !first && j <= a.agg_iters;
             for (;;) {
                 uint32_t qi = 0;
-                if (lane == 0) qi = atomicAdd(&s_qhead, 1u);
+                if (lane_i == 0) qi = atomicAdd(&s_qhead, 1u);
                 qi = (uint32_t)__builtin_amdgcn_readfirstlane((int)qi);
                 if (qi >= qn) break;
                 const uint32_t i = queue[qi];
                 const uint32_t s = cstart[i], e = cstart[i + 1], gs = gstart[i], c = ccell[i];
-                uint32_t rw = lane < (int)kPsRecWords ? recs[(size_t)kPsRecWords * i + lane] : 0u;
+                uint32_t rw = lane_i < (int)kPsRecWords ? recs[(size_t)kPsRecWords * i + lane_i] : 0u;
                 if (skip_mode) {
                     constexpr int32_t ext = (1 << kCellShift) - 1;
                     const uint32_t r1o = (uint32_t)__builtin_amdgcn_readlane((int)rw, 1), pido = (r1o >> 16) & 255u, lpo = r1o >> 24;
@@ -676,8 +685,8 @@
                     if (keep) {
                         Dominance dm;
                         dm.set(bx, ext, npv);
-                        const uint32_t k1 = (uint32_t)lane < nS ? s_mlist[lane] : 0xffffffffu;
-                        const uint32_t ck1 = (uint32_t)lane < nS ? s_mcol[lane] : 0u;
+                        const uint32_t k1 = (uint32_t)lane_i < nS ? s_mlist[lane_i] : 0xffffffffu;
+                        const uint32_t ck1 = (uint32_t)lane_i < nS ? s_mcol[lane_i] : 0u;
                         unsigned long long f1 = __ballot(k1 != 0xffffffffu && dm.worst(ck1) >= 0);
 #pragma unroll
                         for (int w = 0; w < 4; w++)
@@ -691,13 +700,13 @@
                             um[0] |= w == 0 ? bit : 0ull; um[1] |= w == 1 ? bit : 0ull; um[2] |= w == 2 ? bit : 0ull; um[3] |= w == 3 ? bit : 0ull;
                         }
                     } else {
-                        npid = nearest_to_centre(tab, K, bx, ext, lane);
+                        npid = nearest_to_centre(tab, K, bx, ext, lane_i);
                         npv = (uint32_t)__builtin_amdgcn_readfirstlane((int)tab[npid].x);
                         Dominance dm;
                         dm.set(bx, ext, npv);
 #pragma unroll
                         for (int w = 0; w < 4; w++) {
-                            const uint32_t k = 64 * w + lane;
+                            const uint32_t k = 64 * w + lane_i;
                             um[w] = __ballot(k < K && dm.worst(tab[k < K ? k : 0].x) >= 0);
                         }
                         complete = true;
@@ -715,22 +724,22 @@
                     uint32_t nw = rw;
 #pragma unroll
                     for (int t = 0; t < 8; t++)
-                        if (lane == 2 + t) nw = (uint32_t)(um[t >> 1] >> (32 * (t & 1)));
-                    if (lane == 0) nw = npv;
-                    if (lane == 1) nw = r1n;
-                    if (lane == 10) nw = c4;
+                        if (lane_i == 2 + t) nw = (uint32_t)(um[t >> 1] >> (32 * (t & 1)));
+                    if (lane_i == 0) nw = npv;
+                    if (lane_i == 1) nw = r1n;
+                    if (lane_i == 10) nw = c4;
                     rw = nw;
-                    if (lane < (int)kPsRecWords) recs[(size_t)kPsRecWords * i + lane] = rw;
+                    if (lane_i < (int)kPsRecWords) recs[(size_t)kPsRecWords * i + lane_i] = rw;
                     const uint32_t ncd = (uint32_t)(__popcll(um[0]) + __popcll(um[1]) + __popcll(um[2]) + __popcll(um[3]));
                     if (ncd == 1 && (r1o & kPsUlMask) == (c4 & 255u)) continue;
                 }
                 uint32_t wd[kSweep];
                 if (i < Cres) {
 #pragma unroll
-                    for (int u = 0; u < kSweep; u++) { const uint32_t idx = s + u * 64 + lane; wd[u] = idx < e ? pts[idx] : 0u; }
+                    for (int u = 0; u < kSweep; u++) { const uint32_t idx = s + u * 64 + lane_i; wd[u] = idx < e ? pts[idx] : 0u; }
                 } else {
 #pragma unroll
-                    for (int u = 0; u < kSweep; u++) { const uint32_t idx = s + u * 64 + lane; wd[u] = idx < e ? a.pk[gs + (idx - s)] : 0u; }
+                    for (int u = 0; u < kSweep; u++) { const uint32_t idx = s + u * 64 + lane_i; wd[u] = idx < e ? a.pk[gs + (idx - s)] : 0u; }
                 }
                 unsigned long long nm[4];
 #pragma unroll
@@ -749,48 +758,48 @@
                     if (base + 64 * kSweep < e) {
                         if (res) {
 #pragma unroll
-                            for (int u = 0; u < kSweep; u++) { const uint32_t idx = base + 64 * kSweep + u * 64 + lane; w2[u] = idx < e ? pts[idx] : 0u; }
+                            for (int u = 0; u < kSweep; u++) { const uint32_t idx = base + 64 * kSweep + u * 64 + lane_i; w2[u] = idx < e ? pts[idx] : 0u; }
                         } else {
 #pragma unroll
-                            for (int u = 0; u < kSweep; u++) { const uint32_t idx = base + 64 * kSweep + u * 64 + lane; w2[u] = idx < e ? pkc[idx - s] : 0u; }
+                            for (int u = 0; u < kSweep; u++) { const uint32_t idx = base + 64 * kSweep + u * 64 + lane_i; w2[u] = idx < e ? pkc[idx - s] : 0u; }
                         }
                     }
                     if (res) {
                         auto st = [&](uint32_t idx, uint32_t l) { reinterpret_cast<uint8_t *>(pts)[4 * idx + 3] = (uint8_t)l; };
-                        if (first) ps_sweep_first(wd, base, e, s, lane, nm, ncand, cand4, tab, K, cbk, cwc, acc, moved, st);
-                        else uniform = ps_sweep(wd, base, e, s, lane, nm, ncand, cand4, tab, K, cbk, cwc, acc, moved, agg, st) && uniform;
+                        if (first) ps_sweep_first(wd, base, e, s, lane_i, nm, ncand, cand4, tab, K, cbk, cwc, acc, moved, st);
+                        else uniform = ps_sweep(wd, base, e, s, lane_i, nm, ncand, cand4, tab, K, cbk, cwc, acc, moved, agg, st) && uniform;
                     } else {
                         auto st = [&](uint32_t idx, uint32_t l) { reinterpret_cast<uint8_t *>(pkc)[4 * (size_t)(idx - s) + 3] = (uint8_t)l; };
-                        if (first) ps_sweep_first(wd, base, e, s, lane, nm, ncand, cand4, tab, K, cbk, cwc, acc, moved, st);
-                        else uniform = ps_sweep(wd, base, e, s, lane, nm, ncand, cand4, tab, K, cbk, cwc, acc, moved, agg, st) && uniform;
+                        if (first) ps_sweep_first(wd, base, e, s, lane_i, nm, ncand, cand4, tab, K, cbk, cwc, acc, moved, st);
+                        else uniform = ps_sweep(wd, base, e, s, lane_i, nm, ncand, cand4, tab, K, cbk, cwc, acc, moved, agg, st) && uniform;
                     }
 #pragma unroll
                     for (int u = 0; u < kSweep; u++) wd[u] = w2[u];
                 }
-                if (lane == 0) rec[1] = (r1 & ~kPsUlMask) | (uniform && ncand == 1 ? cand4 & 255u : kPsUlMask);
-                evals += (unsigned long long)(e - s) * (ncand + 1);
+                if (lane_i == 0) rec[1] = (r1 & ~kPsUlMask) | (uniform && ncand == 1 ? cand4 & 255u : kPsUlMask);
+                evals += (unsigned long long)(uint32_t)__builtin_amdgcn_readfirstlane((int)(e - s)) * (ncand + 1);
             }
         }
         moved = wave_reduce_sum(moved);
-        if (lane == 0) {
+        if (lane_i == 0) {
             if (moved) atomicAdd(&s_moved, moved);
             if (evals) atomicAdd(&s_evals, evals);
         }
         moved = 0; evals = 0;
         __syncthreads();
-        unsigned long long *Pcur = a.partials + (size_t)(j % 3) * kPsPartWords;
-        for (uint32_t i = tid; i < 5 * K; i += kPsThreads) {
+        unsigned long long *Pcur = ps_partials(a.bar) + (size_t)(j % 3) * kPsPartWords;
+        for (uint32_t i = tid_i; i < 5 * K; i += kPsThreads) {
             const unsigned long long v = acc[i];
             if (v) { __hip_atomic_fetch_add(&Pcur[i], v, __ATOMIC_RELAXED, __HIP_MEMORY_SCOPE_AGENT); acc[i] = 0ull; }
         }
-        if (tid == 0) {
+        if (tid_i == 0) {
             if (s_moved) __hip_atomic_fetch_add(&Pcur[5 * (size_t)K], (unsigned long long)s_moved, __ATOMIC_RELAXED, __HIP_MEMORY_SCOPE_AGENT);
             if (s_evals) __hip_atomic_fetch_add(&Pcur[5 * (size_t)K + 1], s_evals, __ATOMIC_RELAXED, __HIP_MEMORY_SCOPE_AGENT);
             s_moved = 0; s_evals = 0; s_qn = 0; s_qhead = 0; s_nmoved = 0; s_reseed = 0; s_active = 0; s_mm[0] = s_mm[1] = s_mm[2] = s_mm[3] = 0ull;
         }
         asm volatile("s_waitcnt vmcnt(0)" ::: "memory");
         __syncthreads();
-        if (tid == 0) {
+        if (tid_i == 0) {
             bool ok = ps_barrier_xcd(a.bar, ps_xcc_id(), s_nx, s_nxcd, a.timeout_ticks);
 #ifdef CNIIC_TESTING
             if (a.test_abort_at && j + 1 == a.test_abort_at) { ps_st(&a.bar->abort_.v, 1u); ok = false; }
@@ -799,22 +808,23 @@
         }
         __syncthreads();
         if (!s_ok) {
-            if (tid == 0) { a.cold->exit.status = kPsStatusAborted; __threadfence_system(); }
+            if (tid_i == 0) { a.cold->exit.status = kPsStatusAborted; __threadfence_system(); }
             return;
         }
         j++;
         if (blockIdx.x == 0) {
-            unsigned long long *Pclr = a.partials + (size_t)((j + 1) % 3) * kPsPartWords;
-            for (uint32_t i = tid; i < 5 * K + 2; i += kPsThreads) __hip_atomic_store(&Pclr[i], 0ull, __ATOMIC_RELAXED, __HIP_MEMORY_SCOPE_AGENT);
-        }
-        if (tid < K) {
-            const uint32_t k = tid;
+            unsigned long long *Pclr = ps_partials(a.bar) + (size_t)((j + 1) % 3) * kPsPartWords;
+            for (uint32_t i = tid_i; i < 5 * K + 2; i += kPsThreads) __hip_atomic_store(&Pclr[i], 0ull, __ATOMIC_RELAXED, __HIP_MEMORY_SCOPE_AGENT);
+        }
+        if (tid_i < K) {
+            const uint32_t k = tid_i;
             const size_t at[5] = {3 * (size_t)k, 3 * (size_t)k + 1, 3 * (size_t)k + 2, 3 * (size_t)K + k, 4 * (size_t)K + k};
             unsigned long long d[5];
 #pragma unroll
             for (int i = 0; i < 5; i++) d[i] = ps_aread(&Pcur[at[i]]);
-#pragma unroll
-            for (int i = 0; i < 5; i++) run[i] += d[i];
+            unsigned long long run[5];
+#pragma unroll
+            for (int i = 0; i < 5; i++) { run[i] = runs[256 * i + k] + d[i]; runs[256 * i + k] = run[i]; }
             uint32_t ck;
             if (run[4] == 0) {
                 const PsCold *cd = a.cold;
@@ -834,18 +844,18 @@
                 if (pos < kMaxMovedSkip) { s_mlist[pos] = k; s_mcol[pos] = ck; }
                 atomicOr(&s_mm[(k >> 6) & 3], 1ull << (k & 63));
             }
-        } else if (tid == kPsThreads - 1) {
+        } else if (tid_i == kPsThreads - 1) {
             s_changed = ps_aread(&Pcur[5 * (size_t)K]);
             s_pev = ps_aread(&Pcur[5 * (size_t)K + 1]);
         }
         __syncthreads();
         const unsigned long long changed = s_changed;
         nS = s_nmoved;
-        reseeds_total += s_reseed;
-        evals_total += s_pev;
         const bool fin = changed == 0 || (a.max_iters && j >= a.max_iters);
-        if (blockIdx.x == 0 && tid == 0) {
+        if (blockIdx.x == 0 && tid_i == 0) {
             KmDevState *sw = a.st_rw;
+            const unsigned long long reseeds_total = s_rtot + s_reseed, evals_total = s_etot + s_pev;
+            s_rtot = reseeds_total; s_etot = evals_total;
             sw->changed_ring[(j - 1) % kHistRing] = changed;
             sw->nmoved_ring[(j - 1) % kHistRing] = nS;
             if (fin) {
@@ -861,13 +871,14 @@
         const uint2 cc = tab[tid];
         cd->cent_g[tid] = cc.x;
         cd->cconst_g[tid] = cc;
-        cd->members_out[tid] = run[4];
-        cd->wsum_out[tid] = run[3];
-    }
+        cd->members_out[tid] = runs[256 * 4 + tid];
+        cd->wsum_out[tid] = runs[256 * 3 + tid];
+    }
+    uint8_t *labels = dev->p.labels;
     for (uint32_t i = wid; i < C; i += kPsWaves) {
         const uint32_t s = cstart[i], n = cstart[i + 1] - s, gs = gstart[i];
-        if (i < Cres) { for (uint32_t t = lane; t < n; t += 64) a.labels[gs + t] = (uint8_t)(255u - (pts[s + t] >> 24)); }
-        else { for (uint32_t t = lane; t < n; t += 64) a.labels[gs + t] = (uint8_t)(255u - (a.pk[gs + t] >> 24)); }
+        if (i < Cres) { for (uint32_t t = lane; t < n; t += 64) labels[gs + t] = (uint8_t)(255u - (pts[s + t] >> 24)); }
+        else { for (uint32_t t = lane; t < n; t += 64) labels[gs + t] = (uint8_t)(255u - (a.pk[gs + t] >> 24)); }
     }
     if (blockIdx.x == 0) {
         __syncthreads();
@@ -915,20 +926,21 @@
         CNIIC_HIP_TRY(c, hipFuncSetAttribute(reinterpret_cast<const void *>(k_rgbw_persist), hipFuncAttributeMaxDynamicSharedMemorySize, (int)kPsDynBytes));
         attr_set[c->device] = true;
     }
-    const uint64_t o_bar = 0, o_part = (sizeof(PsBar) + 255) & ~255ull, o_fail = o_part + ((3 * (uint64_t)kPsPartWords * 8 + 255) & ~255ull);
-    const uint64_t o_rng = o_fail + 256, total = o_rng + ((uint64_t)G * kPsChunks + 1) * 4;
+    const uint64_t o_part = kPsArenaPart, o_fail = kPsArenaFail, o_rng = kPsArenaRng, total = o_rng + ((uint64_t)G * kPsChunks + 1) * 4;
     CNIIC_HIP_TRY(c, s->ps_arena.alloc(total));
     CNIIC_HIP_TRY(c, hipMemsetAsync(s->ps_arena.p, 0, o_rng, c->stream));
     CNIIC_HIP_TRY(c, s->ps_pk.alloc(std::max<uint64_t>(s->U, 1) * 4));
     s->ps_blocks = G;
     s->ps_o_part = o_part; s->ps_o_fail = o_fail; s->ps_o_rng = o_rng;
-    (void)o_bar;
     uint8_t *a = s->ps_arena.as<uint8_t>();
-    uint32_t budget = kPsDynBytes;
-    if (const char *e = test_env("CNIIC_TEST_PS_LDS_BYTES")) budget = std::min<uint32_t>(kPsDynBytes, (uint32_t)atoi(e));
+    uint32_t budget = kPsBudget;
+    if (const char *e = test_env("CNIIC_TEST_PS_LDS_BYTES")) budget = std::min<uint32_t>(kPsBudget, (uint32_t)atoi(e));
     s->ps_budget = budget;
+    PsDevPtrs ptrs{};
+    ptrs.ckeys = s->ckeys.as<uint32_t>(); ptrs.cweight = s->cweight.as<uint32_t>(); ptrs.labels = s->labels.as<uint8_t>();
+    ptrs.ne_cell = s->ne_cell.as<uint32_t>(); ptrs.ne_start = s->ne_start.as<uint32_t>(); ptrs.cconst0 = s->cconst.as<uint2>();
     hipLaunchKernelGGL(k_ps_ranges, dim3(1), dim3(1024), 0, c->stream, (const uint32_t *)s->ne_cost.as<uint32_t>(), (const uint32_t *)s->ne_count.as<uint32_t>(), G, budget,
-                       reinterpret_cast<uint32_t *>(a + o_rng), reinterpret_cast<uint32_t *>(a + o_fail));
+                       reinterpret_cast<uint32_t *>(a + o_rng), reinterpret_cast<PsDev *>(a + o_fail), ptrs);
     CNIIC_HIP_TRY(c, hipGetLastError());
     s->ps = true;
     return CNIIC_OK;
@@ -949,12 +961,10 @@
     PsExit *xh = &cold->exit;
     uint8_t *ar = s->ps_arena.as<uint8_t>();
     PsArgs a{};
-    a.ckeys = s->ckeys.as<uint32_t>(); a.cweight = s->cweight.as<uint32_t>(); a.labels = s->labels.as<uint8_t>();
-    a.ne_cell = s->ne_cell.as<uint32_t>(); a.ne_start = s->ne_start.as<uint32_t>();
-    a.cb = reinterpret_cast<const uint32_t *>(ar + s->ps_o_rng); a.ranges_fail = reinterpret_cast<const uint32_t *>(ar + s->ps_o_fail);
+    a.cweight = s->cweight.as<uint32_t>();
     a.lds_budget = s->ps_budget;
-    a.pk = s->ps_pk.as<uint32_t>(); a.cconst0 = s->cconst.as<uint2>();
-    a.partials = reinterpret_cast<unsigned long long *>(ar + s->ps_o_part); a.bar = reinterpret_cast<PsBar *>(ar);
+    a.pk = s->ps_pk.as<uint32_t>();
+    a.bar = reinterpret_cast<PsBar *>(ar);
     cold->cconst_g = s->cconst.as<uint2>(); cold->cent_g = s->cent.as<uint32_t>(); cold->members_out = s->members_last.as<uint64_t>(); cold->wsum_out = s->wsum_last.as<uint64_t>();
     cold->keys = s->keys; cold->gx = s->gidx; cold->seed = s->seed; cold->U = s->gidx.bits ? s->gidx.U : s->U;
     a.st_rw = s->dstate.as<KmDevState>(); a.cold = cold; a.max_iters = s->max_iters;
diff --git a/cniic_amd/csrc/kmeans_rgbw.hpp b/cniic_amd/csrc/kmeans_rgbw.hpp
--- a/cniic_amd/csrc/kmeans_rgbw.hpp
+++ b/cniic_amd/csrc/kmeans_rgbw.hpp
@@ -71,10 +71,22 @@
 constexpr uint32_t kPsMaxCells = 2048;
 constexpr uint32_t kPsOffCell = 5 * 256 * 8 + 256 * 8 + kPsSlotsMax * kPsScap * 4;
 constexpr uint32_t kPsDynBytes = 160 * 1024 - 3072;
+constexpr uint32_t kPsRunWords = 5 * 256;
+constexpr uint32_t kPsBudget = kPsDynBytes - kPsRunWords * 8;
 constexpr uint32_t kPsPartWords = 5 * 256 + 8;
 __host__ __device__ constexpr uint32_t ps_cell_bytes(uint32_t C) { return 16u + ((C + 3u) & ~3u) * (4u + 4u + kPsRecWords * 4u + 2u + 2u + 1u); }
+static_assert(kPsOffCell + ps_cell_bytes(kPsMaxCells) <= kPsBudget, "a full block's descriptors fit the budget");
 struct alignas(128) PsLine { uint32_t v; uint32_t pad[31]; };
 struct PsBar { PsLine xcount[8], xgen[8], xblocks[8], top, topgen, count, gen, abort_; };
+struct PsDevPtrs {
+    const uint32_t *ckeys, *cweight;
+    uint8_t *labels;
+    const uint32_t *ne_cell, *ne_start;
+    const uint2 *cconst0;
+};
+struct PsDev { uint32_t fail, pad; PsDevPtrs p; };
+constexpr uint32_t kPsArenaPart = (sizeof(PsBar) + 255u) & ~255u, kPsArenaFail = kPsArenaPart + ((3u * kPsPartWords * 8u + 255u) & ~255u), kPsArenaRng = kPsArenaFail + 256u;
+static_assert(sizeof(PsDev) <= 256, "PsDev has 256 bytes of the arena");
 constexpr uint32_t kPsStatusDone = 1, kPsStatusAborted = 2, kPsStatusRanges = 3;
 struct PsExit { uint32_t status, pad; uint64_t iter, moved_last, reseeds, active, pair_evals; };
 void launch_rgbw_assign_big(Ctx *c, const uint32_t *ckeys, const uint32_t *cweight, uint64_t U, uint32_t K, const uint32_t *cent, uint16_t *labels,
diff --git a/cniic_amd/ps_layout.py b/cniic_amd/ps_layout.py
--- /dev/null
+++ b/cniic_amd/ps_layout.py
@@ -0,0 +1,56 @@
+import numpy as np
+
+PS_CHUNKS = 24
+PS_SLOTS_MAX = 32
+PS_SCAP = 96
+PS_REC_WORDS = 11
+PS_MAX_CELLS = 2048
+PS_OFF_CELL = 5 * 256 * 8 + 256 * 8 + PS_SLOTS_MAX * PS_SCAP * 4
+PS_RUN_BYTES = 5 * 256 * 8
+PS_BUDGET = 160 * 1024 - 3072 - PS_RUN_BYTES
+CELL_FIXED_COST = 512
+CELL_SWEEP_COST = 256
+PS_CELL_DESC_BYTES = 4 + 4 + PS_REC_WORDS * 4 + 2 + 2 + 1
+
+
+def ps_cell_bytes(C):
+    return 16 + ((C + 3) & ~3) * PS_CELL_DESC_BYTES
+
+
+def cell_of(keys):
+    keys = np.asarray(keys, np.uint32)
+    rc, gc, bc = (keys >> 16 & 255) >> 3, (keys >> 8 & 255) >> 3, (keys & 255) >> 3
+    sup = ((rc >> 2) * 8 + (gc >> 2)) * 8 + (bc >> 2)
+    return (sup << 6) | ((rc & 3) << 4) | ((gc & 3) << 2) | (bc & 3)
+
+
+def block_cells(keys, G):
+    counts = np.bincount(cell_of(np.unique(keys)), minlength=32768).astype(np.int64)
+    n = counts[counts > 0]
+    M = n.size
+    sweeps = (n + 255) // 256
+    cost = np.zeros(M + 1, np.int64)
+    cost[1:] = np.cumsum(sweeps) * CELL_SWEEP_COST + np.arange(1, M + 1) * CELL_FIXED_COST
+    NC = G * PS_CHUNKS
+    target = [int(cost[M]) * g // NC for g in range(NC + 1)]
+    cb = np.searchsorted(cost[:M], target, side="left")
+    cb[NC] = M
+    return [np.concatenate([n[cb[r * G + b]:cb[r * G + b + 1]] for r in range(PS_CHUNKS)]) for b in range(G)]
+
+
+def smallest_budget(keys, G, off_cell=PS_OFF_CELL):
+    return off_cell + ps_cell_bytes(max(len(c) for c in block_cells(keys, G)))
+
+
+def resident_points(keys, G, budget=PS_BUDGET, off_cell=PS_OFF_CELL):
+    res = tot = refused = 0
+    for n in block_cells(keys, G):
+        tot += int(n.sum())
+        if len(n) > PS_MAX_CELLS or off_cell + ps_cell_bytes(len(n)) > budget:
+            refused += 1
+            continue
+        cap = (budget - off_cell - ps_cell_bytes(len(n))) // 4
+        ends = np.cumsum(n)
+        fit = int(np.searchsorted(ends, cap, side="right"))
+        res += int(ends[fit - 1]) if fit else 0
+    return res, tot, refused
```

Result: faster. 10300 Mpixels/s (median of 6 runs) (+2.6%).
